# ztaylor797/APMBackend

Measured on AMD Instinct MI355X. Metric: log-lines/sec z-scored (whole node), higher is better.
Workload: dtype fp64

## Files before the change

### apmbackend_amd/csrc/bindings.cpp

```cpp
#include <pybind11/pybind11.h>
#include <pybind11/stl.h>

#include <cstring>
#include <memory>

#include "kernels/kernel_api.h"
#include "runtime/engine.h"
#include "runtime/format.h"
#include "runtime/jsutil.h"
#include "runtime/merge.h"

namespace apm {
namespace copyenc {
void encode_blob(std::string_view blob, std::string* out, int64_t* counts);
}
int apm_txcopy_lines(const char* d_text, const uint64_t* h_line_off, int64_t n, std::string& out_rows);
std::vector<double> apm_release_bench(int64_t n, int iters, uint64_t seed);
}

namespace py = pybind11;
using namespace apm;

void register_tailer(py::module_& m);
void register_synth(py::module_& m);
// ... 42 lines not shown
  c.max_lines = get<uint32_t>(d, "max_lines", c.max_lines);
  c.max_chunks = get<uint32_t>(d, "max_chunks", c.max_chunks);
  c.pool_cap = get<int64_t>(d, "pool_cap", c.pool_cap);
  c.max_tx_per_batch = get<int32_t>(d, "max_tx_per_batch", c.max_tx_per_batch);
  c.max_alerts = get<int32_t>(d, "max_alerts", c.max_alerts);
  c.ring_bytes = get<int>(d, "ring_bytes", c.ring_bytes);
  c.exact_mean = get<int>(d, "exact_mean", c.exact_mean);
  c.sigma_stddev = get<int>(d, "sigma_stddev", c.sigma_stddev);
  c.resync_k = get<int>(d, "resync_k", c.resync_k);
  c.resync_mfma = get<bool>(d, "resync_mfma", c.resync_mfma);
  c.emulate_aliasing = get<int>(d, "emulate_aliasing", c.emulate_aliasing);
  if (d.contains("lags")) {
    auto lags = d["lags"].cast<std::vector<std::tuple<int, double, double>>>();
    c.n_lags = (int)std::min<size_t>(lags.size(), MAX_LAGS);
    for (int i = 0; i < c.n_lags; ++i) {
      c.lags[i] = std::get<0>(lags[i]);
      c.thr[i] = std::get<1>(lags[i]);
      c.infl[i] = std::get<2>(lags[i]);
    }
  }
  if (d.contains("lag_suppressed")) {
    auto v = d["lag_suppressed"].cast<std::vector<int>>();
    for (size_t i = 0; i < v.size() && i < MAX_LAGS; ++i) c.lag_suppressed[i] = v[i];
  }
  c.alert_window = get<int>(d, "alert_window", c.alert_window);
  c.alert_threshold = get<int>(d, "alert_threshold", c.alert_threshold);
  c.hard_min_ms = get<double>(d, "hard_min_ms", c.hard_min_ms);
  c.hard_min_tpm = get<double>(d, "hard_min_tpm", c.hard_min_tpm);
  c.hard_max_ms = get<double>(d, "hard_max_ms", c.hard_max_ms);
  c.both_only = get<int>(d, "both_only", c.both_only);
  c.cooldown_ms = get<double>(d, "cooldown_ms", c.cooldown_ms);
  c.cooldown_by_service = get<int>(d, "cooldown_by_service", c.cooldown_by_service);
  c.alert_clock_entry = get<int>(d, "alert_clock_entry", c.alert_clock_entry);
  c.interval_len = get<int>(d, "interval_len", c.interval_len);
  c.window = get<int>(d, "window", c.window);
  c.buffer = get<int>(d, "buffer", c.buffer);
  c.nslot = get<int>(d, "nslot", c.nslot);
  c.ck_stage_bytes = get<int64_t>(d, "ck_stage_bytes", c.ck_stage_bytes);
  c.record_ttl_ms = get<double>(d, "record_ttl_ms", c.record_ttl_ms);
  c.acct_ttl_ms = get<double>(d, "acct_ttl_ms", c.acct_ttl_ms);
  c.need_ttl_ms = get<double>(d, "need_ttl_ms", c.need_ttl_ms);
  c.tz = tz_from(d);
  c.join_threads = get<int>(d, "join_threads", c.join_threads);
  c.pin_threads = get<bool>(d, "pin_threads", c.pin_threads);
  c.coll_timeout_ms = get<double>(d, "coll_timeout_ms", c.coll_timeout_ms);
  c.coll_init_timeout_ms = get<double>(d, "coll_init_timeout_ms", c.coll_init_timeout_ms);
  c.node_cooldown = get<int>(d, "node_cooldown", c.node_cooldown);
  c.outputs = get<uint32_t>(d, "outputs", c.outputs);
  if (d.contains("win_pcts")) {
    auto v = d["win_pcts"].cast<std::vector<int64_t>>();
    if (v.size() > 8) throw std::invalid_argument("win_pcts: at most 8 percentiles");
    c.n_win_pcts = (int32_t)v.size();
    for (size_t i = 0; i < v.size(); ++i) {
      if (v[i] < 1 || v[i] > 100000 || (i && v[i] <= v[i - 1]))
        throw std::invalid_argument("win_pcts: strictly ascending integers in 1 .. 100000 (percentile * 1000)");
      c.win_pcts[i] = (int32_t)v[i];
    }
  }
  if (d.contains("slo_classes")) {
    c.slo_classes = d["slo_classes"].cast<std::vector<std::vector<int64_t>>>();
    if (d.contains("slo_services")) c.slo_services = d["slo_services"].cast<std::map<std::string, int32_t>>();
    c.slo_default = get<int32_t>(d, "slo_default", 0);
  }
  if (d.contains("svc_pcts")) {
    auto v = d["svc_pcts"].cast<std::vector<int64_t>>();
    if (v.size() > 8) throw std::invalid_argument("svc_pcts: at most 8 percentiles");
    c.n_svc_pcts = (int32_t)v.size();
    for (size_t i = 0; i < v.size(); ++i) {
      if (v[i] < 1 || v[i] > 100000 || (i && v[i] <= v[i - 1]))
        throw std::invalid_argument("svc_pcts: strictly ascending integers in 1 .. 100000 (percentile * 1000)");
      c.svc_pcts[i] = (int32_t)v[i];
    }
  }
  if (d.contains("tk_k") && !d["tk_k"].is_none()) {
    c.tk_k = d["tk_k"].cast<int32_t>();
    if (d.contains("tk_by")) c.tk_by = d["tk_by"].cast<std::vector<int32_t>>();
    c.tk_min_tpm = get<double>(d, "tk_min_tpm", 0.0);
  }
  c.async_stats = get<int>(d, "async_stats", c.async_stats);
  c.device_join = get<int>(d, "device_join", c.device_join);
  c.join_table_bits = get<int>(d, "join_table_bits", c.join_table_bits);
  c.need_arena = get<uint32_t>(d, "need_arena", c.need_arena);
  c.join_chain_blocks = get<uint32_t>(d, "join_chain_blocks", c.join_chain_blocks);
  c.tx_ring_bytes = get<uint64_t>(d, "tx_ring_bytes", c.tx_ring_bytes);
  c.max_raw_services = get<uint32_t>(d, "max_raw_services", c.max_raw_services);
  return c;
}

ServiceOverride override_from(const py::dict& d) {
  ServiceOverride o;
  if (d.contains("thr")) {
    auto v = d["thr"].cast<std::vector<py::object>>();
    for (size_t i = 0; i < v.size() && i < MAX_LAGS; ++i)
      if (!v[i].is_none()) { o.has_thr[i] = true; o.thr[i] = v[i].cast<double>(); }
  }
  if (d.contains("infl")) {
    auto v = d["infl"].cast<std::vector<py::object>>();
    for (size_t i = 0; i < v.size() && i < MAX_LAGS; ++i)
      if (!v[i].is_none()) { o.has_infl[i] = true; o.infl[i] = v[i].cast<double>(); }
  }
  o.hard_max = get<double>(d, "hard_max", 0.0);
  o.suppressed = get<bool>(d, "suppressed", false);
  return o;
}

std::vector<Chunk> chunks_from(const std::vector<std::tuple<int32_t, uint64_t, uint64_t>>& v) {
  std::vector<Chunk> out;
  out.reserve(v.size());
  for (auto& t : v) out.push_back(Chunk{std::get<0>(t), std::get<1>(t), std::get<2>(t)});
  return out;
}

py::dict metrics_dict(const EngineMetrics& m) {
  py::dict d;
  d["batches"] = m.batches; d["bytes"] = m.bytes; d["lines"] = m.lines; d["events"] = m.events;
  d["tx"] = m.tx; d["tx_db"] = m.tx_db; d["tx_dropped"] = m.tx_dropped; d["rollovers"] = m.rollovers;
  d["alerts"] = m.alerts; d["alert_candidates"] = m.alert_candidates;
  d["alert_candidates_dropped"] = m.alert_candidates_dropped; d["released"] = m.released;
  d["staged_batches"] = m.staged_batches;
  d["t_join_shards_ms"] = m.t_join_shards_ms; d["t_merge_ms"] = m.t_merge_ms;
  d["t_shard_busy_ms"] = m.t_shard_busy_ms; d["t_shard_max_ms"] = m.t_shard_max_ms;
  d["t_out_ms"] = m.t_out_ms;
  d["t_lockstep_ms"] = m.t_lockstep_ms; d["t_lockstep_max_ms"] = m.t_lockstep_max_ms;
  d["t_lockstep_stats_ms"] = m.t_lockstep_stats_ms;
  d["db_copy_rows"] = m.db_copy_rows; d["db_copy_fallbacks"] = m.db_copy_fallbacks;
  d["t_stats_tx_ms"] = m.t_stats_tx_ms; d["t_rollover_ms"] = m.t_rollover_ms;
  d["t_format_ms"] = m.t_format_ms; d["t_release_ms"] = m.t_release_ms;
  d["formatted_bytes"] = m.formatted_bytes; d["lockstep_rollovers"] = m.lockstep_rollovers; d["format_fallbacks"] = m.format_fallbacks;
  d["t_parse_ms"] = m.t_parse_ms; d["t_join_ms"] = m.t_join_ms; d["t_stats_ms"] = m.t_stats_ms;
  d["t_total_ms"] = m.t_total_ms;
  d["series_overflow_tx"] = m.series_overflow_tx;
  d["spill_dropped"] = m.spill_dropped;
  d["nan_windows_clipped"] = m.nan_windows_clipped;
  d["tx_capacity_grows"] = m.tx_capacity_grows;
  d["spill_grows"] = m.spill_grows;
  d["spill_capacity"] = m.spill_capacity;
  d["rollover_latency_ms"] = m.rollover_latency_ms;
  return d;
}

py::dict counters_dict(const JoinCounters& c) {
  py::dict d;
  d["events"] = c.events; d["tx"] = c.tx; d["tx_db"] = c.tx_db; d["expired_partials"] = c.expired_partials;
  d["need_expired"] = c.need_expired; d["ejb_exit_unmatched"] = c.ejb_exit_unmatched;
  d["invalid_acct"] = c.invalid_acct; d["audit_errors"] = c.audit_errors; d["host_fallback"] = c.host_fallback;
  d["partial_overflow"] = c.partial_overflow; d["need_overflow"] = c.need_overflow; d["table_full"] = c.table_full;
  d["pool_exhausted"] = c.pool_exhausted; d["chain_partial_blocks"] = c.chain_partial_blocks;
  d["chain_need_blocks"] = c.chain_need_blocks; d["chain_logid_blocks"] = c.chain_logid_blocks;
  d["table_slots"] = c.table_slots; d["table_grows"] = c.table_grows; d["table_rebuilds"] = c.table_rebuilds; d["trims"] = c.trims;
  d["need_arena_entries"] = c.need_arena_entries; d["arena_grows"] = c.arena_grows;
  d["chain_pool_blocks"] = c.chain_pool_blocks; d["pool_grows"] = c.pool_grows;
  d["host_events"] = c.host_events;
  return d;
}

class JoinHarness {
 public:
  explicit JoinHarness(const py::dict& d) {
    cfg_.record_ttl_ms = get<double>(d, "record_ttl_ms", 120000);
    cfg_.acct_ttl_ms = get<double>(d, "acct_ttl_ms", 120000);
    cfg_.need_ttl_ms = get<double>(d, "need_ttl_ms", 30000);
    cfg_.tz = tz_from(d);
  }
  int32_t add_file(const std::string& path, int kind, const std::string& server) {
    int32_t sid;
    auto it = server_ids_.find(server);
    if (it == server_ids_.end()) {
      sid = (int32_t)servers_.size();
      servers_.push_back(server);
      server_ids_[server] = sid;
      shards_.emplace_back(new JoinShard(cfg_, &dict_, &files_, &servers_));
    } else {
      sid = it->second;
    }
    files_.push_back(FileInfo{path, sid, (uint8_t)kind});
    return (int32_t)files_.size() - 1;
  }
  std::vector<std::pair<std::string, std::string>> process(py::bytes events, py::bytes batch,
                                                           std::vector<int32_t> chunk_file, double now) {
    std::string ev = events;
    std::string by = batch;
    const Event* e = reinterpret_cast<const Event*>(ev.data());
    const size_t n = ev.size() / sizeof(Event);
    std::vector<std::pair<uint32_t, uint32_t>> range(shards_.size(), {0, 0});
    uint32_t i = 0;
    while (i < n) {
      const int32_t srv = files_[chunk_file[e[i].chunk]].server;
      uint32_t j = i;
      while (j < n && files_[chunk_file[e[j].chunk]].server == srv) ++j;
      range[srv] = {i, j};
      i = j;
    }
    std::vector<std::pair<std::string, std::string>> out;
    std::vector<TxOut> all;
    for (size_t s = 0; s < shards_.size(); ++s) {
      shards_[s]->out().clear();
      shards_[s]->begin_batch(now, batch_no_);
      if (range[s].second > range[s].first)
        shards_[s]->process(e + range[s].first, range[s].second - range[s].first, (const uint8_t*)by.data(),
                            chunk_file);
      for (auto& t : shards_[s]->out()) all.push_back(t);
    }
// ... 477 lines not shown
        rv.erase(rv.begin() + j);
      }
      if (sv.size() != rv.size() || !std::equal(rv.begin(), rv.end(), sv.begin())) return false;
    }
    return true;
  });
  m.def("gpu_to_fixed", [](const std::vector<double>& xs, int f, const std::string& mode) {
    const int md = mode == "nf" ? 0 : mode == "json" ? 1 : mode == "copy" ? 2 : -1;
    if (md < 0) throw std::invalid_argument("gpu_to_fixed: mode is nf, json or copy");
    if (f != 1 && f != 2) throw std::invalid_argument("gpu_to_fixed: f is 1 or 2");
    const int n = (int)xs.size();
    std::vector<char> h((size_t)n * 32);
    DevMem dx((size_t)n * 8), dout(h.size());
    HIP_OK(hipMemcpy(dx.p, xs.data(), (size_t)n * 8, hipMemcpyHostToDevice));
    apm_format_fixed_batch(dx.as<double>(), n, f, md, dout.as<char>(), 0);
    HIP_OK(hipMemcpy(h.data(), dout.p, h.size(), hipMemcpyDeviceToHost));
    std::vector<std::string> r;
    for (int i = 0; i < n; ++i) r.emplace_back(h.data() + (size_t)i * 32);
    return r;
  }, py::arg("xs"), py::arg("f"), py::arg("mode") = "nf");
  m.def("gpu_fleet_rows", [](const std::vector<double>& moments, const std::vector<std::string>& names,
                             const std::vector<int32_t>& lag_values, int32_t slot_lo, int32_t n_slots, bool copy,
                             int64_t edge_ts) {
    const int n_lags = (int)lag_values.size();
    if (n_lags < 1 || n_lags > MAX_LAGS) throw std::invalid_argument("gpu_fleet_rows: 1..MAX_LAGS lag values");
    if (slot_lo < 0 || n_slots < 0 || (size_t)slot_lo + (size_t)n_slots > names.size())
      throw std::invalid_argument("gpu_fleet_rows: slots outside names");
    if (moments.size() != names.size() * (size_t)n_lags * NSTAT * 3)
      throw std::invalid_argument("gpu_fleet_rows: moments hold names x lags x 3 x 3 doubles");
    std::vector<int32_t> nm;
    std::string chars;
    size_t longest = 0;
    for (const std::string& s : names) {
      nm.push_back((int32_t)chars.size());
      nm.push_back((int32_t)s.size());
      chars += s;
      longest = std::max(longest, s.size());
    }
    const int32_t rows = n_slots * n_lags;
    const uint32_t blocks = apm_fleet_format_blocks(rows);
    const size_t cap = apm_fleet_out_bound(rows, longest);
    DevMem m_mom(moments.size() * 8), m_nm(nm.size() * 4), m_out(cap);
    DevMem m_chars(chars.size() + 64);
    DevMem m_status((size_t)blocks * 8 + 64);
    double* d_mom = m_mom.as<double>();
    int32_t* d_nm = m_nm.as<int32_t>();
    char *d_chars = m_chars.as<char>(), *d_out = m_out.as<char>();
    unsigned long long* d_status = m_status.as<unsigned long long>();
    HIP_OK(hipMemset(d_chars, 0, chars.size() + 64));
    HIP_OK(hipMemset(d_status, 0, (size_t)blocks * 8 + 64));
    HIP_OK(hipMemcpy(d_mom, moments.data(), moments.size() * 8, hipMemcpyHostToDevice));
    HIP_OK(hipMemcpy(d_nm, nm.data(), nm.size() * 4, hipMemcpyHostToDevice));
    if (!chars.empty()) HIP_OK(hipMemcpy(d_chars, chars.data(), chars.size(), hipMemcpyHostToDevice));
    FleetFormatArgs fa{};
    fa.moments = d_mom;
    fa.names = reinterpret_cast<const int2*>(d_nm);
    fa.chars = d_chars;
    fa.slot_lo = slot_lo;
    fa.n_slots = n_slots;
    fa.n_lags = n_lags;
    std::vector<int> order(n_lags);
    for (int l = 0; l < n_lags; ++l) order[l] = l;
    std::sort(order.begin(), order.end(), [&](int a, int b) { return lag_values[a] < lag_values[b]; });
    for (int l = 0; l < n_lags; ++l) { fa.lag_order[l] = order[l]; fa.lag_value[l] = lag_values[l]; }
    fa.edge_ts = edge_ts;
    fa.copy = copy ? 1 : 0;
    fa.ts_len = Engine::pg_timestamp(edge_ts, fa.ts);
    fa.status = d_status;
    fa.total = reinterpret_cast<uint32_t*>(d_status + blocks);
    fa.out = d_out;
    fa.fallback = reinterpret_cast<int32_t*>(d_status + blocks) + 1;
    apm_fleet_format(&fa, 0);
    uint32_t total = 0;
    HIP_OK(hipMemcpy(&total, fa.total, 4, hipMemcpyDeviceToHost));
    if (total > cap) throw std::runtime_error("gpu_fleet_rows: rows longer than the output bound");
    std::string out(total, '\0');
    if (total) HIP_OK(hipMemcpy(&out[0], d_out, total, hipMemcpyDeviceToHost));
    return py::bytes(out);
  }, py::arg("moments"), py::arg("names"), py::arg("lag_values"), py::arg("slot_lo"), py::arg("n_slots"),
     py::arg("copy"), py::arg("edge_ts"));
  m.def("js_to_fixed", [](double x, int f) { return js::to_fixed(x, f); });
  m.def("js_num_str", [](double x) { return js::num_str(x); });
  m.def("js_parse_int", [](const std::string& s) { return js::parse_int(s); });
  m.def("js_convert_date", [](const std::string& s, const py::dict& tz) {
    double v;
    TzTable t = tz_from(tz);
    if (!js::convert_date(s, t, v)) return py::object(py::none());
    return py::object(py::float_(v));
  });
  m.def("js_round_fixed", [](double x, int f) { return js_round_fixed(x, f); });
  m.def("hist_bin", [](int32_t v) { return hist_bin(v); });
  m.def("hist_lower", [](int b) { return hist_lower(b); });
  m.def("hist_group_max", []() { return apm_hist_group_max(); });
  m.def("winpct_group_max", []() { return apm_winpct_group_max(); });
  m.def("winpct_group_win", []() { return apm_winpct_group_win(); });
  m.def("slo_group_max", []() { return apm_slo_group_max(); });
  m.def("slo_stage_bytes", []() { return apm_slo_stage_bytes(); });
  m.def("svcwin_group_max", []() { return apm_svcwin_group_max(); });
  m.def("svcwin_group_win", []() { return apm_svcwin_group_win(); });
  m.def("apm_topk_tile", []() { return apm_topk_tile(); });
  m.def("apm_topk_final_span", []() { return apm_topk_final_span(); });
  m.def("topk_select", [](const std::vector<std::tuple<double, double, double, double, int32_t>>& win_rows,
                          const std::vector<int32_t>& perm, int32_t k, const std::vector<int32_t>& by, double min_tpm) {
    if (k < 1 || k > TK_MAX_K) throw std::invalid_argument("topk_select: k is 1 .. 128");
    if (by.empty() || by.size() > (size_t)TK_MAX_BOARDS) throw std::invalid_argument("topk_select: 1 to 4 boards");
    for (int32_t c : by)
      if (c < TK_TPM || c > TK_P95) throw std::invalid_argument("topk_select: keys are 0 .. 3");
    for (int32_t s : perm)
      if (s < 0 || (size_t)s >= win_rows.size()) throw std::invalid_argument("topk_select: perm names no series");
    const int32_t n = (int32_t)perm.size(), S = (int32_t)win_rows.size(), nb = (int32_t)by.size();
    std::vector<WinStat> win((size_t)S);
    for (int32_t s = 0; s < S; ++s) {
      win[s].tpm = std::get<0>(win_rows[s]); win[s].avg = std::get<1>(win_rows[s]);
      win[s].p75 = std::get<2>(win_rows[s]); win[s].p95 = std::get<3>(win_rows[s]);
      win[s].n = 0; win[s].active = std::get<4>(win_rows[s]);
    }
    DevMem dwin((size_t)S * sizeof(WinStat)), dperm((size_t)n * 4), dsc(apm_topk_scratch_bytes(n, k, nb));
    DevMem dout((size_t)nb * k * sizeof(TopKRec)), dn(64);
    if (S) HIP_OK(hipMemcpy(dwin.p, win.data(), (size_t)S * sizeof(WinStat), hipMemcpyHostToDevice));
    if (n) HIP_OK(hipMemcpy(dperm.p, perm.data(), (size_t)n * 4, hipMemcpyHostToDevice));
    TopKArgs a{};
    a.win = dwin.as<WinStat>(); a.perm = dperm.as<int32_t>(); a.n = n; a.n_series = S; a.k = k; a.nb = nb;
    for (int32_t b = 0; b < nb; ++b) a.by[b] = by[b];
    a.min_tpm = min_tpm;
    a.out = dout.as<TopKRec>(); a.out_n = dn.as<int32_t>();
    apm_topk(&a, dsc.p, 0);
    std::vector<TopKRec> rec((size_t)nb * k);
    int32_t cnt[TK_MAX_BOARDS] = {0, 0, 0, 0};
    HIP_OK(hipMemcpy(cnt, dn.p, (size_t)nb * 4, hipMemcpyDeviceToHost));
    HIP_OK(hipMemcpy(rec.data(), dout.p, rec.size() * sizeof(TopKRec), hipMemcpyDeviceToHost));
    py::list out;
    for (int32_t b = 0; b < nb; ++b) {
      py::list rows;
      for (int32_t r = 0; r < std::min(std::max(cnt[b], 0), k); ++r)
        rows.append(py::make_tuple(rec[(size_t)b * k + r].series, rec[(size_t)b * k + r].pos));
      out.append(rows);
    }
    return out;
  }, py::arg("win_rows"), py::arg("perm"), py::arg("k"), py::arg("by"), py::arg("min_tpm") = 0.0);

  register_tailer(m);
  register_synth(m);
  register_procstat(m);
  register_dbsink(m);
}
```

### apmbackend_amd/csrc/kernels/kernel_api.h

```cpp
#pragma once
#include <hip/hip_runtime.h>
#include <stdint.h>

#include "../apm_types.h"
#include "common.h"

namespace apm {

struct StatsState {
  int32_t* counts;
  int32_t* cells;
  int32_t* spill_n;
  int32_t* spill_series;
  int32_t* spill_val;
  uint8_t* active;
  int32_t cap;
  int32_t spill_cap;
  int32_t S;
  int32_t nslot = NSLOT_MIN;
  unsigned long long* spill_drop = nullptr;
  int32_t* nan_until = nullptr;
  int32_t* ord_list = nullptr;
  int32_t* ord_n = nullptr;
  uint32_t* ord_done = nullptr;
// ... 205 lines not shown
struct TopKRec {
  int32_t series, pos;
  WinStat w;
};
struct TopKArgs {
  const WinStat* win;
  const int32_t* perm;
  int32_t n;
  int32_t n_series;
  int32_t k;
  int32_t nb;
  int32_t by[TK_MAX_BOARDS];
  double min_tpm;
  TopKRec* out;
  int32_t* out_n;
  int32_t tiles;
  uint64_t* sc_key;
  int32_t* sc_pos;
};
struct SvcRec {
  int32_t servers;
  int32_t m, nan;
  int32_t first_pos;
  long long sum;
  long long sum2[WP_MAX_Q];
};
struct SvcWinArgs {
  WindowArgs w;
  int32_t nq;
  int32_t q[WP_MAX_Q];
  int32_t n_groups;
  const int32_t* grp_off;
  const int32_t* grp_mem;
  const int32_t* grp_pos;
  SvcRec* rec;
  int32_t* big_list;
  int32_t* big_n;
};
struct SvcWinTextArgs {
  const SvcRec* rec;
  const int32_t* series_grp;
  const int32_t* perm;
  const int4* series_names;
  const char* names;
  int32_t n;
  int32_t n_series;
  int32_t n_groups;
  int32_t nq;
  int32_t ts_len;
  char ts[24];
  char ptxt[WP_MAX_Q][8];
  int32_t plen[WP_MAX_Q];
  uint32_t *len, *off;
  char* out;
};
struct AlertArgs {
  const WinStat* win;
  const ZOut* z;
  int32_t* counter;
  const double* hard_max;
  const uint8_t* suppressed;
  const uint64_t* emit_key;
  AlertRec* out;
  int32_t* n_out;
  int32_t n_series;
  int32_t lag_idx;
  int32_t n_lags;
  int32_t lag_suppressed;
  int32_t window;
  int32_t threshold;
  double hard_min_ms;
  double hard_min_tpm;
  int32_t both_only;
  int32_t max_out;
  const double* cool_t;
  double now;
  double cool_s;
};

}

extern "C" {
size_t apm_parse_workspace_bytes(uint64_t max_bytes, uint32_t max_lines, uint32_t max_chunks);
int apm_parse_batch(const uint8_t* d_bytes, uint64_t n_bytes, const uint32_t* d_chunk_begin,
                    const uint8_t* d_chunk_kind, const uint32_t* d_chunk_file, uint32_t n_chunks,
                    void* d_ws, uint32_t max_lines, apm::Event* d_events, uint32_t* d_n_events,
                    uint32_t* d_n_lines, unsigned long long* d_watermark, uint8_t* d_file_open,
                    const apm::TzTable* tz, hipStream_t stream);
size_t apm_ck_pack_tmp_bytes(uint64_t n_entries);
int apm_ck_pack_cells(const int32_t* counts, const int32_t* cells, const int32_t* d_slots, int k, int32_t n, int32_t S,
                      int32_t cap, uint32_t* lens, uint32_t* offs, void* tmp, size_t tmp_bytes, int32_t* packed,
                      hipStream_t s);
void apm_stats_clear_slot(apm::StatsState* st, int slot, hipStream_t stream);
void apm_bucket_append(const apm::TxRec* d_tx, uint32_t lo, uint32_t hi, apm::StatsState* st,
                       int64_t min_live_bucket, hipStream_t stream);
void apm_nan_mark(const apm::TxRec* d_tx, uint32_t n, apm::StatsState* st, hipStream_t stream);
void apm_window_stats(apm::WindowArgs* a, hipStream_t stream);
size_t apm_spill_sort_tmp_bytes(int32_t spill_cap, int32_t S, int32_t nslot);
int apm_spill_sort(const apm::StatsState* st, int32_t* series_out, int32_t* val_out, void* tmp, size_t tmp_bytes,
                   hipStream_t stream);
void apm_pool_append(const apm::TxRec* d_tx, uint32_t lo, uint32_t hi, const int64_t* d_gid, int64_t* tail_end,
                     int64_t* tail_gid, int64_t base, hipStream_t stream);
size_t apm_release_tmp_bytes(int64_t cap);
int apm_release_merge(const int64_t* pool_end, const int64_t* pool_gid, int64_t n_pool, const int64_t* tail_end,
                      const int64_t* tail_gid, int64_t n_tail, int64_t* sort_end, int64_t* sort_gid,
                      int64_t* out_end, int64_t* out_gid, void* tmp, size_t tmp_bytes, hipStream_t stream);
void apm_export(const apm::ExportArgs* a, hipStream_t stream);
void apm_copy(void* dst, const void* src, size_t bytes, hipStream_t stream);
void apm_copy_capped(void* dst, const void* src, size_t bytes, uint32_t max_blocks, hipStream_t stream);
void apm_copy_segs(const apm::CopySegs* c, hipStream_t stream);
void apm_set_f64(double* dst, const double* vals, int n, hipStream_t stream);
void apm_zscore(apm::ZArgs* a, int dtype_bytes, hipStream_t stream);
void apm_zscore_warm(apm::ZArgs* a, int dtype_bytes, int fill, uint64_t seed, const apm::WinStat* base,
                     hipStream_t stream);
void apm_server_rollup(apm::RollupArgs* a, hipStream_t stream);
size_t apm_format_tmp_bytes(int32_t n_max);
void apm_format_fixed_batch(const double* d_x, int n, int f, int mode, char* d_out, hipStream_t stream);
int apm_format_plan(apm::FormatArgs* a, void* tmp, size_t tmp_bytes, hipStream_t stream);
void apm_format_write(apm::FormatArgs* a, hipStream_t stream);
void apm_alert_eval(apm::AlertArgs* a, hipStream_t stream);
void apm_scatter_f64(double* dst, const int32_t* idx, const double* val, int32_t n, hipStream_t stream);
uint32_t apm_fleet_format_blocks(int32_t n_rows);
size_t apm_fleet_out_bound(int32_t rows, size_t longest);
void apm_fleet_format(apm::FleetFormatArgs* a, hipStream_t stream);
void apm_alert_gather(const apm::AlertRec* alerts, const int32_t* n_dev, int32_t max_n, const apm::WinStat* win,
                      const apm::ZOut* const* z_by_lag, int32_t n_lags, int32_t rows, apm::AlertRec* alerts_out,
                      apm::WinStat* win_out, apm::ZOut* z_out, int32_t* n_out, hipStream_t stream);
int32_t apm_hist_group_max();
size_t apm_hist_tmp_bytes(int32_t n_max);
size_t apm_hist_row_bound(size_t name_bytes);
int apm_hist_plan(apm::HistArgs* a, void* tmp, size_t tmp_bytes, hipStream_t stream);
void apm_hist_write(apm::HistArgs* a, hipStream_t stream);
int32_t apm_winpct_group_max();
int32_t apm_winpct_group_win();
size_t apm_winpct_tmp_bytes(int32_t n_max);
size_t apm_winpct_row_bound(size_t name_bytes, int32_t nq);
void apm_winpct_values(apm::WinPctArgs* a, hipStream_t stream);
int apm_winpct_plan(apm::WinPctTextArgs* a, void* tmp, size_t tmp_bytes, hipStream_t stream);
void apm_winpct_write(apm::WinPctTextArgs* a, hipStream_t stream);
int32_t apm_slo_group_max();
int32_t apm_slo_stage_bytes();
size_t apm_slo_tmp_bytes(int32_t n_max);
size_t apm_slo_row_bound(size_t name_bytes);
void apm_slo_values(apm::SloArgs* a, hipStream_t stream);
int apm_slo_plan(apm::SloTextArgs* a, void* tmp, size_t tmp_bytes, hipStream_t stream);
void apm_slo_write(apm::SloTextArgs* a, hipStream_t stream);
int32_t apm_topk_tile();
int32_t apm_topk_final_span();
size_t apm_topk_scratch_bytes(int32_t n_max, int32_t k, int32_t nb);
void apm_topk(apm::TopKArgs* a, void* scratch, hipStream_t stream);
int32_t apm_svcwin_group_max();
int32_t apm_svcwin_group_win();
size_t apm_svcwin_tmp_bytes(int32_t n_max);
size_t apm_svcwin_row_bound(size_t name_bytes, int32_t nq);
void apm_svcwin_values(apm::SvcWinArgs* a, hipStream_t stream);
int apm_svcwin_plan(apm::SvcWinTextArgs* a, void* tmp, size_t tmp_bytes, hipStream_t stream);
void apm_svcwin_write(apm::SvcWinTextArgs* a, hipStream_t stream);
void apm_service_moments(const int32_t* series_service, const uint8_t* active, int32_t n_series, int32_t S,
                         int32_t n_lags, int32_t n_services_cap, const double* const* sums, const double* const* comps,
                         const int32_t* const* cnts, double* dst, hipStream_t stream);
void apm_service_moments_tail(const int32_t* series_service, const uint8_t* active, int32_t s_lo, int32_t n_series,
                              int32_t S, int32_t n_lags, int32_t n_services_cap, const double* const* sums,
                              const double* const* comps, const int32_t* const* cnts, double* dst,
                              hipStream_t stream);
int apm_service_gram(const int32_t* svc_off, const int32_t* svc_ids, const uint8_t* active, int32_t n_services,
                     int32_t S, int32_t n_lags, const double* const* sums, const double* const* comps,
                     const int32_t* const* cnts, double* dst, hipStream_t stream, const int32_t* svc_map = nullptr,
                     int32_t accumulate = 0);
}
```

### apmbackend_amd/csrc/kernels/parse.hip

```cpp
#include "kernel_api.h"

#include "prim.h"

#include "devscan.h"

#include <algorithm>
#include <cstdio>
#include <cstdlib>
#include <cstring>

namespace apm {

constexpr int NL_BLOCK = 256;
constexpr int NL_TILE = NL_BLOCK * 16;
constexpr int PARSE_BLOCK = 256;
constexpr int PARSE_LDS = 32 * 1024;

constexpr int NL_PER = 4;

__device__ __forceinline__ uint32_t nl_count16(const uint4 v) {
  const uint32_t w[4] = {v.x, v.y, v.z, v.w};
  uint32_t c = 0;
#pragma unroll
  for (int k = 0; k < 4; ++k) {
    const uint32_t x = w[k] ^ 0x0a0a0a0aU;
    const uint32_t t = ~(((x & 0x7F7F7F7Fu) + 0x7F7F7F7Fu) | x | 0x7F7F7F7Fu);
    c += __popc(t);
  }
  return c;
}

__global__ __launch_bounds__(NL_BLOCK) void k_nl_count(const uint8_t* __restrict__ bytes, uint64_t n,
                                                      uint32_t* __restrict__ tile_counts, uint8_t* __restrict__ pad,
                                                      uint32_t tiles) {
  if (blockIdx.x == 0 && threadIdx.x < 64) pad[threadIdx.x] = 0;
  if (blockIdx.x == 0 && threadIdx.x == 64) tile_counts[tiles] = 0;
  uint4 v[NL_PER];
  uint64_t base[NL_PER];
#pragma unroll
  for (int k = 0; k < NL_PER; ++k) {
    base[k] = ((uint64_t)blockIdx.x * NL_PER + k) * NL_TILE + threadIdx.x * 16;
    if (base[k] + 16 <= n) v[k] = *reinterpret_cast<const uint4*>(bytes + base[k]);
  }
  uint32_t pk[NL_PER / 2] = {0, 0};
#pragma unroll
  for (int k = 0; k < NL_PER; ++k) {
    uint32_t c = 0;
    if (base[k] + 16 <= n) {
      c = nl_count16(v[k]);
    } else {
      for (uint64_t i = base[k]; i < n && i < base[k] + 16; ++i) c += bytes[i] == '\n';
    }
    pk[k >> 1] += c << (16 * (k & 1));
  }
  __shared__ uint32_t red[NL_PER / 2][NL_BLOCK / APM_WAVE];
#pragma unroll
  for (int h = 0; h < NL_PER / 2; ++h) {
    uint32_t c = pk[h];
    for (int o = 32; o > 0; o >>= 1) c += __shfl_down(c, o, APM_WAVE);
    if ((threadIdx.x & 63) == 0) red[h][threadIdx.x >> 6] = c;
  }
  __syncthreads();
  if (threadIdx.x < NL_PER) {
    const int k = threadIdx.x;
    uint32_t sum = 0;
    for (int i = 0; i < NL_BLOCK / APM_WAVE; ++i) sum += red[k >> 1][i];
    const uint32_t tile = blockIdx.x * NL_PER + k;
    if (tile < tiles) tile_counts[tile] = (sum >> (16 * (k & 1))) & 0xFFFFu;
  }
}

__global__ __launch_bounds__(NL_BLOCK) void k_nl_write(const uint8_t* __restrict__ bytes, uint64_t n,
                                                      const uint32_t* __restrict__ tile_off,
                                                      uint32_t* __restrict__ line_end, uint32_t* __restrict__ n_lines,
                                                      uint32_t tiles) {
  if (blockIdx.x == 0 && threadIdx.x == 0) *n_lines = tile_off[tiles];
  uint4 v[NL_PER];
#pragma unroll
  for (int k = 0; k < NL_PER; ++k) {
    const uint64_t base = ((uint64_t)blockIdx.x * NL_PER + k) * NL_TILE + threadIdx.x * 16;
    v[k] = base + 16 <= n ? *reinterpret_cast<const uint4*>(bytes + base) : make_uint4(0, 0, 0, 0);
  }
  typedef rocprim::block_scan<int, NL_BLOCK> Scan;
  __shared__ typename Scan::storage_type st;
#pragma unroll
  for (int k = 0; k < NL_PER; ++k) {
    const uint32_t tile = blockIdx.x * NL_PER + k;
    if (tile >= tiles) break;
    const uint64_t base = (uint64_t)tile * NL_TILE + threadIdx.x * 16;
    uint8_t b[16];
    if (base + 16 <= n) {
      const uint32_t w[4] = {v[k].x, v[k].y, v[k].z, v[k].w};
#pragma unroll
      for (int q = 0; q < 4; ++q) {
#pragma unroll
        for (int j = 0; j < 4; ++j) b[q * 4 + j] = (uint8_t)(w[q] >> (8 * j));
      }
    } else {
      for (int i = 0; i < 16; ++i) b[i] = (base + i < n) ? bytes[base + i] : 0;
    }
    int c = 0;
#pragma unroll
    for (int i = 0; i < 16; ++i) c += b[i] == '\n';
    int excl;
    Scan().exclusive_scan(c, excl, 0, st);
    uint32_t pos = tile_off[tile] + excl;
#pragma unroll
    for (int i = 0; i < 16; ++i)
      if (b[i] == '\n') line_end[pos++] = (uint32_t)(base + i);
    __syncthreads();
  }
}

__device__ __forceinline__ bool is_ws(uint8_t c) {
  return c <= 32 && ((0x100003E00ULL >> c) & 1ULL);
}
__device__ __forceinline__ bool is_digit(uint8_t c) { return c >= '0' && c <= '9'; }
__device__ __forceinline__ uint8_t lower(uint8_t c) { return (c >= 'A' && c <= 'Z') ? c + 32 : c; }

template <int N>
__device__ __forceinline__ bool match_at(const uint8_t* p, int i, int len, const char (&lit)[N]) {
  if (i + N - 1 > len) return false;
#pragma unroll
  for (int k = 0; k < N - 1; ++k)
    if (p[i + k] != (uint8_t)lit[k]) return false;
  return true;
}

constexpr int NTOKSLOT = 7;
__device__ __forceinline__ constexpr int tok_slot(int k) {
  return k <= 3 ? k : (k == 9 ? 4 : (k == 11 ? 5 : (k == 13 ? 6 : 0)));
}
__device__ __forceinline__ void tok_put(uint16_t (&arr)[NTOKSLOT], int k, uint16_t v) {
  constexpr int idx[NTOKSLOT] = {0, 1, 2, 3, 9, 11, 13};
#pragma unroll
  for (int j = 0; j < NTOKSLOT; ++j) arr[j] = k == idx[j] ? v : arr[j];
}
__device__ __forceinline__ void tok_put_if(uint16_t (&arr)[NTOKSLOT], bool on, int k, uint16_t v) {
  tok_put(arr, on ? k : -1, v);
}
constexpr uint64_t kTokSlotTab = 0xFF6F5F4FFFFF3210ULL;
__device__ __forceinline__ int tok_slot_of(int k) { return k < 16 ? (int)((kTokSlotTab >> (4 * k)) & 0xFu) : 15; }

template <int N>
__device__ __forceinline__ constexpr uint32_t pk4(const char (&lit)[N]) {
  static_assert(N == 5, "pk4 takes exactly four characters");
  return (uint32_t)(uint8_t)lit[0] | ((uint32_t)(uint8_t)lit[1] << 8) | ((uint32_t)(uint8_t)lit[2] << 16) |
         ((uint32_t)(uint8_t)lit[3] << 24);
}

__device__ __forceinline__ uint32_t swar_eq(uint32_t d, uint32_t k4) {
  const uint32_t x = d ^ k4;
  return ~(((x & 0x7F7F7F7Fu) + 0x7F7F7F7Fu) | x | 0x7F7F7F7Fu);
}
__device__ __forceinline__ uint32_t swar_ws(uint32_t d) {
  const uint32_t y = d & 0x7F7F7F7Fu;
  const uint32_t rng = (y + 0x77777777u) & ~(y + 0x72727272u) & ~d & 0x80808080u;
  return rng | swar_eq(d, 0x20202020u);
}
__device__ __forceinline__ uint32_t swar_bits(uint32_t t) { return (((t >> 7) * 0x00204081u) >> 21) & 0xFu; }

struct Masks16 {
  uint32_t ws, na, trig;
};
__device__ __forceinline__ Masks16 masks16(const uint32_t (&d)[5]) {
  Masks16 r{0u, 0u, 0u};
#pragma unroll
  for (int q = 0; q < 4; ++q) {
    r.ws |= swar_bits(swar_ws(d[q])) << (4 * q);
    r.na |= swar_bits(d[q] & 0x80808080u) << (4 * q);
// ... 22 lines not shown
  if (i < e && (p[i] == '+' || p[i] == '-')) { neg = p[i] == '-'; ++i; }
  if (i + 1 < e && p[i] == '0' && (p[i + 1] == 'x' || p[i + 1] == 'X')) return false;
  int64_t v = 0;
  int nd = 0;
  while (i < e && is_digit(p[i])) {
    v = v * 10 + (p[i] - '0');
    ++i;
    if (++nd > 15) return false;
  }
  out = nd == 0 ? apm_nan() : (neg ? -(double)v : (double)v);
  return true;
}

__device__ inline bool parse_log_ts(const uint8_t* p, int s1, int e1, int s2, int e2,
                                    const TzTable& tz, double& out, bool& strict) {
  int64_t v[8];
  int np = 0;
  int nd[8];
  strict = false;
  for (int pass = 0; pass < 2; ++pass) {
    const int s = pass ? s2 : s1, e = pass ? e2 : e1;
    int64_t cur = 0;
    int cnt = 0;
    for (int i = s; i <= e; ++i) {
      const bool end = i == e;
      const uint8_t c = end ? '-' : p[i];
      if (c == '-' || c == ':' || c == ',') {
        if (np >= 8) return false;
        v[np] = cur; nd[np] = cnt; ++np;
        cur = 0; cnt = 0;
        if (end) break;
      } else if (is_digit(c)) {
        cur = cur * 10 + (c - '0');
        if (++cnt > 12) return false;
      } else {
        return false;
      }
    }
  }
  if (np < 7) {
    out = apm_nan();
    return np >= 2;
  }
  const int64_t yr = (v[0] >= 0 && v[0] <= 99) ? v[0] + 1900 : v[0];
  const int64_t local = make_date_ms(yr, v[1] - 1, v[2], v[3], v[4], v[5], v[6]);
  out = (double)local_to_utc(tz, local);
  strict = np == 7 && nd[0] == 4 && nd[1] == 2 && nd[2] == 2 && nd[3] == 2 && nd[4] == 2 &&
           nd[5] == 2 && nd[6] >= 1 && nd[6] <= 3;
  return true;
}

__device__ __forceinline__ bool parse_log_ts_fixed(const uint8_t* p, int s1, int e1, int s2, int e2,
                                                   const TzTable& tz, double& out) {
  if (e1 - s1 != 10 || e2 - s2 != 12) return false;
  uint32_t a[10], b[12];
#pragma unroll
  for (int k = 0; k < 10; ++k) a[k] = (uint32_t)p[s1 + k] - '0';
#pragma unroll
  for (int k = 0; k < 12; ++k) b[k] = (uint32_t)p[s2 + k] - '0';
  bool ok = a[4] == (uint32_t)('-' - '0') && a[7] == (uint32_t)('-' - '0') && b[2] == (uint32_t)(':' - '0') &&
            b[5] == (uint32_t)(':' - '0') && b[8] == (uint32_t)(',' - '0');
  constexpr int da[8] = {0, 1, 2, 3, 5, 6, 8, 9};
  constexpr int db[9] = {0, 1, 3, 4, 6, 7, 9, 10, 11};
#pragma unroll
  for (int k = 0; k < 8; ++k) ok &= a[da[k]] <= 9u;
#pragma unroll
  for (int k = 0; k < 9; ++k) ok &= b[db[k]] <= 9u;
  if (!ok) return false;
  const int64_t y = a[0] * 1000 + a[1] * 100 + a[2] * 10 + a[3];
  const int64_t mo = a[5] * 10 + a[6], d = a[8] * 10 + a[9];
  const int64_t h = b[0] * 10 + b[1], mi = b[3] * 10 + b[4], sec = b[6] * 10 + b[7];
  const int64_t ms = b[9] * 100 + b[10] * 10 + b[11];
  const int64_t yr = y <= 99 ? y + 1900 : y;
  out = (double)local_to_utc(tz, make_date_ms(yr, mo - 1, d, h, mi, sec, ms));
  return true;
}

struct ParseArgs {
  const uint8_t* bytes;
  const uint32_t* line_end;
  const uint32_t* chunk_begin;
  const uint8_t* chunk_kind;
  const uint32_t* n_lines_dev;
  uint32_t cap_lines;
  uint32_t n_chunks;
  Event* ev_tmp;
  uint32_t* line_mask;
  uint8_t* keep;
  unsigned long long* watermark;
  unsigned long long* prof;
  TzTable tz;
};

enum : int { PP_STAGE = 0, PP_SCAN, PP_HITS, PP_LINES, PP_WAVES, PP_COOP, PP_SERIAL, PP_HEAD, PP_TAIL, PP_N = 10 };
__device__ __forceinline__ void pprof(const ParseArgs& a, int k, long long& t) {
  if (a.prof) {
    const long long now = clock64();
    if ((threadIdx.x & (APM_WAVE - 1)) == 0) atomicAdd(&a.prof[k], (unsigned long long)(now - t));
    t = now;
  }
}

__device__ __forceinline__ uint32_t find_chunk_in(const uint32_t* cb, uint32_t lo, uint32_t hi, uint32_t pos) {
  while (lo < hi) {
    uint32_t mid = (lo + hi + 1) >> 1;
    if (cb[mid] <= pos) lo = mid; else hi = mid - 1;
  }
  return lo;
}

__device__ __forceinline__ uint32_t find_chunk(const uint32_t* cb, uint32_t n_chunks, uint32_t pos) {
  uint32_t lo = 0, hi = n_chunks - 1;
  while (lo < hi) {
    uint32_t mid = (lo + hi + 1) >> 1;
    if (cb[mid] <= pos) lo = mid; else hi = mid - 1;
  }
  return lo;
}

template <int STRIDE = PARSE_BLOCK>
__device__ __forceinline__ unsigned long long parse_line(const ParseArgs& a, const uint8_t* __restrict__ base,
                                                         uint32_t o, uint32_t li, uint32_t ls, uint32_t le,
                                                         uint32_t c_lo, uint32_t c_hi, uint16_t* tp);

enum : uint32_t { XF_EJB_ENTRY = 1, XF_EJB_EXIT = 2, XF_CT_START = 4, XF_CT_STOP = 8, XF_BAF = 16, XF_NONASCII = 32 };

template <class P>
__device__ __forceinline__ void probe_flags(P p, int len, int s, uint32_t& m, uint32_t& xf) {
  const uint32_t w4 = (uint32_t)p[s] | ((uint32_t)p[s + 1] << 8) | ((uint32_t)p[s + 2] << 16) |
                      ((uint32_t)p[s + 3] << 24);
  if (w4 == pk4("INFO")) {
    int j = s + 4;
    while (j < len && p[j] == ' ') ++j;
    if (match_at(p, j, len, "[CommonTiming] The EJB")) xf |= XF_EJB_ENTRY;
    if (match_at(p, j, len, "[CommonTiming] Total time")) xf |= XF_EJB_EXIT;
    if (match_at(p, j, len, "CommonTiming::Start")) xf |= XF_CT_START;
    if (match_at(p, j, len, "CommonTiming::Stop")) xf |= XF_CT_STOP;
    if (match_at(p, s, len, "INFO  auditTrailId=")) m |= PM_AUTR_MAP;
    if (!(xf & XF_BAF) && s + 4 < len && p[s + 4] == ' ' && s >= 1 && p[s - 1] == ' ') {
      int kk0 = s - 1;
      while (kk0 >= 0 && p[kk0] == ' ') --kk0;
      if (kk0 >= 0 && p[kk0] == ']')
        for (int kk = kk0 - 2; kk >= 0 && p[kk] != ' '; --kk)
          if (p[kk] == '[') { xf |= XF_BAF; break; }
    }
    return;
  }
  if (w4 == pk4(": Re")) {
    if (match_at(p, s, len, ": RequestTrace [stopWatchList=")) m |= PM_EL_START;
    return;
  }
  if ((w4 & 0xffu) != '<') return;
  const uint32_t w4l = (uint32_t)lower(p[s]) | ((uint32_t)lower(p[s + 1]) << 8) |
                       ((uint32_t)lower(p[s + 2]) << 16) | ((uint32_t)lower(p[s + 3]) << 24);
  if (w4 == pk4("<sto")) {
    if (match_at(p, s, len, "<stopWatchList>")) m |= PM_SW_START;
    if (match_at(p, s, len, "<stopTime>")) m |= PM_SW_STOPTS;
  } else if (w4 == pk4("</st")) {
    if (match_at(p, s, len, "</stopWatchList>")) m |= PM_SW_END;
  } else if (w4 == pk4("<nam")) {
    if (match_at(p, s, len, "<name>")) m |= PM_SW_NAME;
  } else if (w4 == pk4("<sta")) {
    if (match_at(p, s, len, "<startTime>")) m |= PM_SW_STARTTS;
  } else if (w4 == pk4("<val")) {
    if (match_at(p, s, len, "<value>")) m |= PM_SOAP_VALUE;
  }
  if (w4l == pk4("<acc")) {
    if (match_at_ci(p, s, len, "<accountnumber>")) m |= PM_SOAP_ACCT;
  } else if (w4l == pk4("<key")) {
    if (match_at_ci(p, s, len, "<key>accountnumber</key>")) m |= PM_SOAP_KEY;
  }
}

template <int STRIDE>
__device__ __forceinline__ unsigned long long line_tail(const ParseArgs& a, const uint8_t* __restrict__ p, int len,
                                                        uint32_t li, Event& ev, uint8_t fk, int ntok, uint32_t m,
                                                        uint32_t xf, int info1, int info2, const uint16_t* tp,
                                                        int bias);
__device__ __forceinline__ bool line_head(const ParseArgs& a, const uint8_t* __restrict__ p, uint32_t li,
                                          uint32_t ls, uint32_t le, uint32_t c_lo, uint32_t c_hi, Event& ev,
                                          uint8_t& fk, int& len);

__global__ __launch_bounds__(PARSE_BLOCK) void k_parse_lines(ParseArgs a) {
  __shared__ __attribute__((aligned(16))) uint8_t lds[PARSE_LDS];
  __shared__ uint16_t tok_lds[2 * NTOKSLOT][PARSE_BLOCK];
  long long pt = a.prof ? clock64() : 0;
  const uint32_t n_lines = *a.n_lines_dev;
  const uint32_t first = blockIdx.x * PARSE_BLOCK;
  if (first >= n_lines) {
    const uint32_t li = first + threadIdx.x;
    if (li < a.cap_lines) a.keep[li] = 0;
    return;
  }
  const uint32_t last = min(first + PARSE_BLOCK, n_lines);
  const uint32_t r0 = first == 0 ? 0 : a.line_end[first - 1] + 1;
  const uint32_t r1 = a.line_end[last - 1] + 1;
  const uint32_t a0 = r0 & ~15u;
  const uint32_t span = r1 - a0;
  const bool staged = span <= PARSE_LDS;
  if (staged) {
    const uint32_t nvec = (span + 15) >> 4;
    const uint4* __restrict__ src = reinterpret_cast<const uint4*>(a.bytes + a0);
    uint4* dst = reinterpret_cast<uint4*>(lds);
    const uint32_t t = threadIdx.x;
    for (uint32_t i = t; i < nvec; i += 4 * PARSE_BLOCK) {
      const bool b1 = i + PARSE_BLOCK < nvec, b2 = i + 2 * PARSE_BLOCK < nvec, b3 = i + 3 * PARSE_BLOCK < nvec;
      const uint4 v0 = src[i];
      const uint4 v1 = b1 ? src[i + PARSE_BLOCK] : v0;
      const uint4 v2 = b2 ? src[i + 2 * PARSE_BLOCK] : v0;
      const uint4 v3 = b3 ? src[i + 3 * PARSE_BLOCK] : v0;
      dst[i] = v0;
      if (b1) dst[i + PARSE_BLOCK] = v1;
      if (b2) dst[i + 2 * PARSE_BLOCK] = v2;
      if (b3) dst[i + 3 * PARSE_BLOCK] = v3;
    }
  }
  __syncthreads();
  pprof(a, PP_STAGE, pt);
  const uint32_t li = first + threadIdx.x;
  unsigned long long wm = 0;
  if (li >= last) {
    if (li < a.cap_lines) a.keep[li] = 0;
  } else {
    const uint32_t ls = li == 0 ? 0 : a.line_end[li - 1] + 1;
    const uint32_t le = a.line_end[li];
    const uint32_t c_lo = find_chunk(a.chunk_begin, a.n_chunks, r0), c_hi = find_chunk(a.chunk_begin, a.n_chunks, r1 - 1);
    wm = staged ? parse_line<PARSE_BLOCK>(a, lds, ls - a0, li, ls, le, c_lo, c_hi, &tok_lds[0][threadIdx.x])
                : parse_line<PARSE_BLOCK>(a, a.bytes, ls, li, ls, le, c_lo, c_hi, &tok_lds[0][threadIdx.x]);
  }
  if (a.prof) {
    pprof(a, PP_LINES, pt);
    if ((threadIdx.x & (APM_WAVE - 1)) == 0) atomicAdd(&a.prof[PP_WAVES], 1ull);
  }
  for (int off = APM_WAVE / 2; off > 0; off >>= 1) {
    const unsigned long long o2 = __shfl_xor(wm, off, APM_WAVE);
    wm = o2 > wm ? o2 : wm;
  }
  if ((threadIdx.x & (APM_WAVE - 1)) == 0 && wm) atomicMax(a.watermark, wm);
}

__device__ __forceinline__ bool line_head(const ParseArgs& a, const uint8_t* __restrict__ p, uint32_t li,
                                          uint32_t ls, uint32_t le, uint32_t c_lo, uint32_t c_hi, Event& ev,
                                          uint8_t& fk, int& len) {
  len = (int)(le - ls);
  if (len > 0 && p[len - 1] == '\r') --len;

  ev.line = li;
  ev.chunk = find_chunk_in(a.chunk_begin, c_lo, c_hi, ls);
  ev.off = ls;
  ev.len = (uint32_t)len;
  ev.mask = 0;
  ev.kind = LK_NONE;
  ev.ntok = 0;
  ev.pad0 = 0;
  ev.t0s = ev.t0e = ev.t1s = ev.t1e = ev.t2s = ev.t2e = ev.t3s = ev.t3e = 0xffff;
  ev.tAs = ev.tAe = ev.tBs = ev.tBe = 0xffff;
  ev.ts = apm_nan();
  ev.num = apm_nan();
  ev.key = 0;
  ev.svc = 0;
  fk = a.chunk_kind[ev.chunk];
  if (len <= 0 || len > 65000) {
    a.keep[li] = (len > 65000) ? 1 : 0;
    if (len > 65000) { ev.kind = fk == FILE_SOAP ? LK_SOAP : LK_APP; ev.mask = PM_HOST; }
    a.line_mask[li] = ev.mask;
    a.ev_tmp[li] = ev;
    return false;
  }
  return true;
}

constexpr int TILE = NL_TILE;
constexpr int TSTAGE = TILE + 1024;
constexpr int TMAXL = 128;
constexpr int THITS = 256;

__device__ __forceinline__ uint32_t tscan_op(uint32_t x, uint32_t y) {
  const uint32_t ls = (x & 0x1FFFu) + (y & 0x1FFFu);
  const uint32_t hits = (x >> 19) + (y >> 19);
  uint32_t seg, has;
  if (y & 0x2000u) {
    seg = (y >> 14) & 31u;
    has = 1u;
  } else {
    seg = min(((x >> 14) & 31u) + ((y >> 14) & 31u), 31u);
    has = (x >> 13) & 1u;
  }
  return ls | (has << 13) | (seg << 14) | (hits << 19);
}

__global__ __launch_bounds__(APM_WAVE) void k_parse_tiles(ParseArgs a, uint64_t n, const uint32_t* __restrict__ tile_off) {
  __shared__ __attribute__((aligned(16))) uint8_t st[TSTAGE + 32];
  __shared__ uint16_t tok[2 * NTOKSLOT][TMAXL];
  __shared__ uint16_t c_ls[TMAXL], c_le[TMAXL];
  __shared__ uint8_t c_nt[TMAXL];
  __shared__ uint32_t c_m[TMAXL], c_xf[TMAXL], c_i1[TMAXL], c_i2[TMAXL];
  __shared__ uint32_t hit[THITS];
  const int lane = threadIdx.x;
  long long pt = a.prof ? clock64() : 0;
  const uint32_t n_lines = *a.n_lines_dev;
  for (uint32_t li = n_lines + blockIdx.x * APM_WAVE + lane; li < a.cap_lines; li += gridDim.x * APM_WAVE)
    a.keep[li] = 0;
  const uint64_t T0 = (uint64_t)blockIdx.x * TILE;
  if (T0 >= n) return;
  const uint64_t T1 = min(T0 + TILE, n);
  const bool own0 = T0 == 0 || a.bytes[T0 - 1] == '\n';
// ... 473 lines not shown
    const unsigned long long cm = __ballot(is_close);
    const unsigned long long below = lane ? ((1ULL << lane) - 1ULL) : 0ULL;
    const unsigned long long ob = om & below, cb = cm & below;
    bool in;
    if (!ob && !cb) in = open;
    else {
      const int lo_ = ob ? 63 - __clzll(ob) : -1;
      const int lc_ = cb ? 63 - __clzll(cb) : -1;
      in = lo_ > lc_;
    }
    if (valid && in && !is_open) {
      line_mask[li] = m | PM_IN_SECTION;
      if (!keep[li]) {
        keep[li] = 1;
        ev_tmp[li].kind = LK_APP;
      }
      ev_tmp[li].mask |= PM_IN_SECTION;
    }
    const unsigned long long all = om | cm;
    if (all) {
      const int l = 63 - __clzll(all);
      open = (om >> l) & 1ULL;
    }
  }
  if (g == SEC_SEGS - 1 && lane == 0) {
    bool fin = chunk_init[c] != 0;
    for (int h = SEC_SEGS - 1; h >= 0; --h) {
      const uint8_t st = seg_state[(size_t)c * SEC_SEGS + h];
      if (st) { fin = st == 1; break; }
    }
    file_open[chunk_file[c]] = fin ? 1 : 0;
  }
}

__global__ void k_chunk_lines(const uint32_t* __restrict__ chunk_begin, uint32_t n_chunks,
                              const uint32_t* __restrict__ line_end, const uint32_t* __restrict__ n_lines_dev,
                              uint32_t* __restrict__ chunk_line_lo, const uint32_t* __restrict__ tile_off,
                              uint32_t tiles) {
  const uint32_t c = blockIdx.x * blockDim.x + threadIdx.x;
  if (c > n_chunks) return;
  const uint32_t n_lines = *n_lines_dev;
  const uint32_t pos = chunk_begin[c];
  const uint32_t t = pos / (uint32_t)NL_TILE;
  uint32_t lo = t < tiles ? tile_off[t] : n_lines, hi = t < tiles ? tile_off[t + 1] : n_lines;
  while (lo < hi) {
    uint32_t mid = (lo + hi) >> 1;
    if (line_end[mid] < pos) lo = mid + 1; else hi = mid;
  }
  chunk_line_lo[c] = lo;
}

struct KeepF {
  const uint8_t* keep;
  __device__ uint32_t operator()(uint32_t i) const { return keep[i]; }
};
struct CompactG {
  const uint8_t* keep;
  const Event* ev_tmp;
  Event* out;
  __device__ void operator()(uint32_t i, uint32_t p) const {
    if (keep[i]) out[p] = ev_tmp[i];
  }
};

}

extern "C" {

constexpr size_t APM_SCAN_TMP = 32u << 20;

size_t apm_parse_workspace_bytes(uint64_t max_bytes, uint32_t max_lines, uint32_t max_chunks) {
  using namespace apm;
  const uint64_t tiles = (max_bytes + NL_TILE - 1) / NL_TILE + 2;
  size_t b = 0;
  b += tiles * 8 + 64;
  b += (size_t)max_lines * (4 + 4 + 4 + 1) + 64;
  b += (size_t)max_lines * sizeof(Event) + 64;
  b += (size_t)(max_chunks + 2) * 4 + 256;
  b += (size_t)(max_chunks + 2) * (SEC_SEGS + 1) + 256;
  b += APM_SCAN_TMP;
  return b;
}

int apm_parse_batch(const uint8_t* d_bytes, uint64_t n_bytes, const uint32_t* d_chunk_begin,
                    const uint8_t* d_chunk_kind, const uint32_t* d_chunk_file, uint32_t n_chunks,
                    void* d_ws, uint32_t max_lines, apm::Event* d_events, uint32_t* d_n_events,
                    uint32_t* d_n_lines, unsigned long long* d_watermark, uint8_t* d_file_open,
                    const apm::TzTable* tz, hipStream_t stream) {
  using namespace apm;
  const uint32_t tiles = (uint32_t)((n_bytes + NL_TILE - 1) / NL_TILE);
  if (tiles == 0 || n_chunks == 0) {
    HIP_OK(hipMemsetAsync(d_n_events, 0, 4, stream));
    HIP_OK(hipMemsetAsync(d_n_lines, 0, 4, stream));
    HIP_OK(hipMemsetAsync(const_cast<uint8_t*>(d_bytes) + n_bytes, 0, 64, stream));
    return 0;
  }
  const uint32_t cap = (uint32_t)std::min<uint64_t>(max_lines, n_bytes);
  uint8_t* w = (uint8_t*)d_ws;
  auto carve = [&](size_t bytes) { uint8_t* r = (uint8_t*)(((uintptr_t)w + 63) & ~(uintptr_t)63); w = r + bytes; return r; };
  uint32_t* tile_counts = (uint32_t*)carve((size_t)(tiles + 1) * 4);
  uint32_t* tile_off = (uint32_t*)carve((size_t)(tiles + 1) * 4);
  uint32_t* line_end = (uint32_t*)carve((size_t)max_lines * 4);
  Event* ev_tmp = (Event*)carve((size_t)max_lines * sizeof(Event));
  uint32_t* line_mask = (uint32_t*)carve((size_t)max_lines * 4);
  uint32_t* pos = (uint32_t*)carve((size_t)max_lines * 4);
  uint8_t* keep = carve((size_t)max_lines);
  uint32_t* chunk_line_lo = (uint32_t*)carve((size_t)(n_chunks + 2) * 4);
  uint8_t* seg_state = carve((size_t)(n_chunks + 2) * SEC_SEGS);
  uint8_t* chunk_init = carve((size_t)(n_chunks + 2));
  void* scan_tmp = carve(APM_SCAN_TMP);

  const uint32_t nl_blocks = (tiles + NL_PER - 1) / NL_PER;
  hipLaunchKernelGGL(k_nl_count, dim3(nl_blocks), dim3(NL_BLOCK), 0, stream, d_bytes, n_bytes, tile_counts,
                     const_cast<uint8_t*>(d_bytes) + n_bytes, tiles);
  PrimScratch sc(scan_tmp, APM_SCAN_TMP);
  if (prim_exclusive_scan(sc, tile_counts, tile_off, 0u, (size_t)tiles + 1, rocprim::plus<uint32_t>(), stream) != 0)
    return -1;
  hipLaunchKernelGGL(k_nl_write, dim3(nl_blocks), dim3(NL_BLOCK), 0, stream, d_bytes, n_bytes, tile_off, line_end,
                     d_n_lines, tiles);

  ParseArgs pa;
  pa.bytes = d_bytes;
  pa.line_end = line_end;
  pa.chunk_begin = d_chunk_begin;
  pa.chunk_kind = d_chunk_kind;
  pa.n_lines_dev = d_n_lines;
  pa.cap_lines = cap;
  pa.n_chunks = n_chunks;
  pa.ev_tmp = ev_tmp;
  pa.line_mask = line_mask;
  pa.keep = keep;
  pa.watermark = d_watermark;
  pa.tz = *tz;
  static unsigned long long* d_prof = nullptr;
  static int prof_batches = 0;
  static const bool prof_on = getenv("APM_PARSE_PROF") != nullptr;
  if (prof_on && !d_prof) {
    HIP_OK(hipMalloc((void**)&d_prof, PP_N * 8));
    HIP_OK(hipMemsetAsync(d_prof, 0, PP_N * 8, stream));
  }
  pa.prof = prof_on ? d_prof : nullptr;
  const char* mode_env = getenv("APM_PARSE");
  const bool by_line = !(mode_env && strcmp(mode_env, "tile") == 0);
  if (by_line)
    hipLaunchKernelGGL(k_parse_lines, dim3((cap + PARSE_BLOCK - 1) / PARSE_BLOCK), dim3(PARSE_BLOCK), 0,
                       stream, pa);
  else
    hipLaunchKernelGGL(k_parse_tiles, dim3(tiles), dim3(APM_WAVE), 0, stream, pa, n_bytes, (const uint32_t*)tile_off);
  if (prof_on && ++prof_batches % 50 == 0) {
    unsigned long long h[PP_N];
    HIP_OK(hipMemcpyAsync(h, d_prof, sizeof h, hipMemcpyDeviceToHost, stream));
    HIP_OK(hipStreamSynchronize(stream));
    const double w = h[PP_WAVES] ? (double)h[PP_WAVES] : 1.0;
    fprintf(stderr, "[parse prof %s] %d batches, %.0f waves/batch; cycles per wave: stage %.0f scan %.0f hits %.0f "
            "lines %.0f; lines coop %llu serial %llu; per coop line: head %.0f tail %.0f\n", by_line ? "line" : "tile",
            prof_batches, w / prof_batches, h[PP_STAGE] / w, h[PP_SCAN] / w, h[PP_HITS] / w, h[PP_LINES] / w,
            (unsigned long long)h[PP_COOP], (unsigned long long)h[PP_SERIAL],
            h[PP_COOP] ? (double)h[PP_HEAD] / h[PP_COOP] : 0.0, h[PP_COOP] ? (double)h[PP_TAIL] / h[PP_COOP] : 0.0);
  }
  hipLaunchKernelGGL(k_chunk_lines, dim3((n_chunks + 1 + 255) / 256), dim3(256), 0, stream, d_chunk_begin,
                     n_chunks, line_end, d_n_lines, chunk_line_lo, tile_off, tiles);
  hipLaunchKernelGGL(k_section_summary, dim3(n_chunks, SEC_SEGS), dim3(APM_WAVE), 0, stream, chunk_line_lo,
                     d_chunk_kind, d_chunk_file, n_chunks, line_mask, d_file_open, seg_state, chunk_init);
  hipLaunchKernelGGL(k_section_apply, dim3(n_chunks, SEC_SEGS), dim3(APM_WAVE), 0, stream, chunk_line_lo,
                     d_chunk_kind, d_chunk_file, n_chunks, line_mask, keep, ev_tmp, d_file_open, seg_state,
                     chunk_init);
  if (ds_scan_apply<uint32_t>(KeepF{keep}, CompactG{keep, ev_tmp, d_events}, d_n_lines, cap, pos, d_n_events,
                              stream) != 0)
    return -1;
  return 0;
}

}
```

### apmbackend_amd/csrc/runtime/devjoin.h

```cpp
#pragma once
#include <hip/hip_runtime.h>

#include <atomic>
#include <cstdint>
#include <deque>
#include <functional>
#include <mutex>
#include <string>
#include <unordered_map>
#include <vector>

#include "../apm_types.h"
#include "../kernels/devjoin_api.h"
#include "hipres.h"
#include "join.h"

namespace apm {

struct CopySegs;

struct DevJoinConfig {
  uint32_t max_events = 1u << 20;
  uint64_t max_batch_bytes = 64ull << 20;
  uint32_t max_chunks = 4096;
  int table_bits = 21;
  int reg_bits = 20;
  uint32_t max_raw = 1u << 20;
  uint32_t arena_cap = 1u << 20;
  uint32_t pool_blocks = 0;
  uint64_t ring_bytes = 4ull << 30;
  double record_ttl_ms = 120000, acct_ttl_ms = 120000, need_ttl_ms = 30000;
  TzTable tz{};
  int device = 0;
};

struct DevJoinBatch {
  int slot = 0;
  uint32_t n_out = 0, n_stats = 0, n_db = 0, n_dropped = 0;
  std::vector<std::pair<uint32_t, int64_t>> cands;
  std::vector<std::pair<uint32_t, int32_t>> unresolved;
  std::string text_tx, text_db;
  uint64_t ring_base = 0;
  int64_t max_bucket = INT64_MIN;
  TxRec* d_tx = nullptr;
  int32_t* d_raw = nullptr;
  int64_t* d_gid = nullptr;
};

class DeviceJoin {
 public:
  DeviceJoin(const DevJoinConfig& cfg, Dictionary* dict, const std::vector<FileInfo>* files,
             const std::vector<std::string>* servers);
  ~DeviceJoin();

  uint8_t* d_bytes(int k) { return sl_[k].d_bytes; }
  uint8_t* d_stage() {
    if (!d_stage_bytes_) {
      d_stage_bytes_ = (uint8_t*)res_.dmalloc_on(stream_, cfg_.max_batch_bytes + 256);
      HIP_OK(hipStreamSynchronize(stream_));
    }
    return d_stage_bytes_;
  }
  void swap_stage(int k) { std::swap(sl_[k].d_bytes, d_stage_bytes_); }
  Event* d_events(int k) { return sl_[k].d_events; }
  void select_host(int k, const uint32_t* d_n_ev, uint32_t max_ev, hipStream_t ps);
  void set_chunks(int k, const std::vector<int32_t>& chunk_file, const uint32_t* d_chunk_file,
                  const uint8_t* d_chunk_kind);
  void chunk_upload(int k, uint32_t max_ev, CopySegs& cs);
  void export_select(int k, CopySegs& cs);
  using ParallelFor = std::function<void(int, const std::function<void(int)>&)>;
  void run(int k, const uint8_t* host_bytes, uint32_t n_ev, uint64_t n_bytes, double now, uint64_t batch_no, bool want_tx,
           bool want_db, DevJoinBatch& out, const ParallelFor& parallel = nullptr,
           const std::function<void()>* meanwhile = nullptr);
  void prepass_ahead(int k, const uint8_t* host_bytes, const ParallelFor& parallel);
  void release_slot(int k, hipStream_t stats_stream);

  int32_t raw_server(int32_t raw) const { return raw_info_[raw].server; }
  int32_t raw_service(int32_t raw) const { return raw_info_[raw].norm_id; }
  int32_t n_raw() const { return n_raw_.load(std::memory_order_acquire); }
  int32_t* d_raw_series() { return d_raw_series_; }

  char* ring() { return d_ring_; }
  uint64_t ring_cap() const { return cfg_.ring_bytes; }
  void set_ring_low(uint64_t low);
  uint64_t ring_head() const { return ring_head_.load(std::memory_order_acquire); }
  uint64_t ring_low() const { return ring_low_.load(std::memory_order_acquire); }
  uint64_t keys_live() const { return keys_live_ + keys_since_rebuild_; }
  uint64_t need_live() const { return arena_head_ - (regions_.empty() ? arena_head_ : regions_.front().lo); }
  uint64_t ring_reserve(uint64_t bytes);
  void reset_ring(uint64_t head);

  JoinCounters counters() const;
  std::vector<uint64_t> cache_stats(double now, bool sync = true);

  void save(class BinWriter& w);
  void load(class BinReader& r);
  static constexpr int kPhases = 8;
  double phase_t[kPhases + 1] = {0};
  std::vector<std::pair<const char*, std::pair<double, double>>> spans;
  std::vector<std::pair<const char*, std::pair<double, double>>> save_spans;
  const JoinCounts& last_counts() const { return *h_counts_; }
  size_t device_bytes() const { return res_.device_bytes(); }
  size_t trim(double now);

 private:
  struct Slot {
    uint8_t* d_bytes = nullptr;
    Event* d_events = nullptr;
    uint8_t* host_flag = nullptr;
    uint32_t* d_mh_idx = nullptr;
    uint32_t* d_walk_idx = nullptr;
    AudF* d_aud = nullptr;
    SelCount* d_n_host = nullptr;
    Mapped<Event> h_host_ev;
    Mapped<uint32_t> h_host_idx;
    Mapped<SelCount> h_n_host;
    int32_t* d_chunk_next = nullptr;
    uint8_t* d_chunk_first = nullptr;
    Mapped<int32_t> h_chunk_next;
    Mapped<uint8_t> h_chunk_first;
    const uint32_t* d_chunk_file = nullptr;
    const uint8_t* d_chunk_kind = nullptr;
    uint32_t n_chunks = 0;
    std::vector<int32_t> chunk_file;
    TxRec* d_tx = nullptr;
    int32_t* d_tx_raw = nullptr;
    int64_t* d_tx_gid = nullptr;
    hipEvent_t free_ev = nullptr;
    bool used = false;
  } sl_[2];

  struct RawInfo { int32_t server; int32_t norm_id; uint64_t svc; };

  struct PrepassTask {
    int32_t file = -1;
    std::vector<uint32_t> idx;
    std::vector<HostOp> hops;
    std::string hbuf;
    uint64_t audit_errors = 0, invalid_acct = 0, pm_host = 0;
    uint32_t put(std::string_view s) { const uint32_t o = (uint32_t)hbuf.size(); hbuf.append(s.data(), s.size()); return o; }
  };
  void host_prepass(int k, const uint8_t* host_bytes, uint32_t n_host, const ParallelFor& parallel,
                    std::vector<HostOp>& hops, std::string& hbuf);
  void host_event(PrepassTask& t, const Event& e, uint32_t ev, const uint8_t* host_bytes);
  void on_app(PrepassTask& t, const Event& e, uint32_t ev, std::string_view line);
  void save_tables(class BinWriter& w);
  void aud_reserve(AudGen& g, uint32_t autr, uint32_t items, uint64_t txt);
// ... 161 lines not shown
```

### apmbackend_amd/csrc/runtime/engine.cpp

```cpp
#include <cstdlib>
#include "engine.h"

#include <pthread.h>
#include <sched.h>

#include <cctype>
#include <fstream>

#include <rocprofiler-sdk-roctx/roctx.h>

#include <unistd.h>

#include <cerrno>
#include <cstring>

#include <algorithm>
#include <exception>
#include <chrono>
#include <cmath>
#include <cstring>
#include <queue>
#include <stdexcept>

#include "../kernels/devjoin_api.h"
// ... 163 lines not shown
  done_cv_.wait(lk, [&]() { return done_ == n_tasks_; });
  fn_ = nullptr;
  lk.unlock();
  if (err) std::rethrow_exception(err);
}

Engine::Engine(const EngineConfig& cfg) : cfg_(cfg) {
  check_window(cfg_.window, cfg_.buffer, cfg_.interval_len);
  if (cfg_.n_lags < 1 || cfg_.n_lags > MAX_LAGS)
    throw std::runtime_error("engine: 1.." + std::to_string(MAX_LAGS) + " LAG settings");
  if (want(OUT_WP)) {
    const int nq = cfg_.n_win_pcts;
    bool ok = nq >= 1 && nq <= WP_MAX_Q;
    for (int j = 0; ok && j < nq; ++j)
      ok = cfg_.win_pcts[j] >= 1 && cfg_.win_pcts[j] <= 100000 && (j == 0 || cfg_.win_pcts[j] > cfg_.win_pcts[j - 1]);
    if (!ok) throw std::invalid_argument("wp stream: win_pcts must hold 1 to 8 strictly ascending percentiles");
  }
  if (want(OUT_SL)) {
    const auto& cl = cfg_.slo_classes;
    bool ok = !cl.empty() && cl[0].empty() && cl.size() <= (size_t)cfg_.max_series + 2;
    bool any = false;
    for (size_t c = 1; ok && c < cl.size(); ++c) {
      ok = !cl[c].empty() && cl[c].size() <= (size_t)SL_MAX_T;
      for (size_t j = 0; ok && j < cl[c].size(); ++j)
        ok = cl[c][j] >= 0 && cl[c][j] <= INT32_MAX && (j == 0 || cl[c][j] > cl[c][j - 1]);
      any = true;
    }
    const auto in_range = [&](int32_t c) { return c >= 0 && (size_t)c < cl.size(); };
    ok = ok && any && in_range(cfg_.slo_default);
    for (const auto& kv : cfg_.slo_services) ok = ok && in_range(kv.second);
    if (!ok)
      throw std::invalid_argument("sl stream: slo_classes must hold the empty class 0 and at least one class of 1 to 8 "
                                  "strictly ascending thresholds in 0 .. 2147483647; every class index must name one");
  }
  if (want(OUT_TK)) {
    bool ok = cfg_.tk_k >= 1 && cfg_.tk_k <= TK_MAX_K && !cfg_.tk_by.empty() && cfg_.tk_by.size() <= (size_t)TK_MAX_BOARDS &&
              std::isfinite(cfg_.tk_min_tpm) && cfg_.tk_min_tpm >= 0.0;
    for (size_t i = 0; ok && i < cfg_.tk_by.size(); ++i) {
      ok = cfg_.tk_by[i] >= TK_TPM && cfg_.tk_by[i] <= TK_P95;
      for (size_t j = 0; ok && j < i; ++j) ok = cfg_.tk_by[j] != cfg_.tk_by[i];
    }
    if (!ok)
      throw std::invalid_argument("tk stream: tk_k must lie in 1 .. 128, tk_by hold 1 to 4 distinct keys out of "
                                  "0 .. 3 and tk_min_tpm be finite and >= 0");
  }
  if (want(OUT_SV)) {
    const int nq = cfg_.n_svc_pcts;
    bool ok = nq >= 1 && nq <= WP_MAX_Q;
    for (int j = 0; ok && j < nq; ++j)
      ok = cfg_.svc_pcts[j] >= 1 && cfg_.svc_pcts[j] <= 100000 && (j == 0 || cfg_.svc_pcts[j] > cfg_.svc_pcts[j - 1]);
    if (!ok) throw std::invalid_argument("sv stream: svc_pcts must hold 1 to 8 strictly ascending percentiles");
  }
  HIP_OK(hipSetDevice(cfg_.device));
  {
    const char* e = std::getenv("APM_BLOCKING_SYNC");
    if (e && e[0] == '1') (void)hipSetDeviceFlags(hipDeviceScheduleBlockingSync);
  }
  {
    const char* e = std::getenv("APM_CU_RESERVE");
    int n_cu = 0;
    HIP_OK(hipDeviceGetAttribute(&n_cu, hipDeviceAttributeMultiprocessorCount, cfg_.device));
    const int reserve = e ? std::atoi(e) : 0;
    if (reserve > 0 && reserve < n_cu / 2) {
      const int stride = n_cu / reserve;
      std::vector<uint32_t> mask((size_t)(n_cu + 31) / 32, 0u);
      for (int c = 0; c < n_cu; ++c)
        if (c % stride != stride - 1) mask[(size_t)c / 32] |= 1u << (c % 32);
      for (hipStream_t* s : {&stream_, &parse_stream_, &out_stream_})
        HIP_OK(hipExtStreamCreateWithCUMask(s, (uint32_t)mask.size(), mask.data()));
      cu_reserved_ = reserve;
    } else {
      static const bool sp = [] { const char* x = std::getenv("APM_STATS_PRIO"); return !(x && x[0] == '0'); }();
      int lo = 0, hi = 0;
      HIP_OK(hipDeviceGetStreamPriorityRange(&lo, &hi));
      HIP_OK(hipStreamCreateWithPriority(&stream_, hipStreamNonBlocking, sp ? hi : 0));
      static const bool pp = [] { const char* x = std::getenv("APM_PARSE_PRIO"); return x && x[0] == '1'; }();
      HIP_OK(hipStreamCreateWithPriority(&parse_stream_, hipStreamNonBlocking, pp ? hi : 0));
      HIP_OK(hipStreamCreateWithFlags(&out_stream_, hipStreamNonBlocking));
    }
    for (hipStream_t st : {stream_, parse_stream_, out_stream_}) res_.adopt(st);
  }
  ev_a_ = res_.new_event();
  ev_b_ = res_.new_event();
  const int32_t S = cfg_.max_series;
  if (cfg_.device_join) {
    DevJoinConfig dc;
    dc.max_events = cfg_.max_lines;
    dc.max_batch_bytes = cfg_.max_batch_bytes;
    dc.max_chunks = cfg_.max_chunks;
    dc.table_bits = cfg_.join_table_bits;
    dc.max_raw = cfg_.max_raw_services;
    dc.arena_cap = cfg_.need_arena;
    dc.pool_blocks = cfg_.join_chain_blocks;
    dc.ring_bytes = cfg_.tx_ring_bytes;
    dc.record_ttl_ms = cfg_.record_ttl_ms;
    dc.acct_ttl_ms = cfg_.acct_ttl_ms;
    dc.need_ttl_ms = cfg_.need_ttl_ms;
    dc.tz = cfg_.tz;
    dc.device = cfg_.device;
    dj_.reset(new DeviceJoin(dc, &dict_, &files_, &servers_));
    d_ring_min_ = (unsigned long long*)res_.dmalloc(64);
    HIP_OK(hipMemset(d_ring_min_, 0xff, 8));
    res_.pin(h_ring_min_, 64);
    *h_ring_min_ = ~0ULL;
    d_rel_n_ = (int64_t*)res_.dmalloc(64);
    res_.pin(h_rel_n_, 64);
    d_rel_lens_ = (uint32_t*)res_.dmalloc(((size_t)cfg_.pool_cap + 2) * 4);
    d_rel_offs_ = (uint32_t*)res_.dmalloc(((size_t)cfg_.pool_cap + 2) * 4);
    d_rel_fb_ = (uint32_t*)res_.dmalloc(4);
    HIP_OK(hipMemset(d_rel_fb_, 0, 4));
    res_.pin(h_rel_total_, 64);
    d_unmapped_ = (unsigned long long*)res_.dmalloc(64);
    d_unseen_idx_ = (int32_t*)res_.dmalloc((size_t)cfg_.max_series * 4);
    d_unseen_flag_ = (uint8_t*)res_.dmalloc((size_t)cfg_.max_series);
    res_.pin(h_unseen_flag_, (size_t)cfg_.max_series);
  } else {
    d_bytes_ = (uint8_t*)res_.dmalloc(cfg_.max_batch_bytes + 256);
  }
  for (int k = 0; k < 2; ++k) {
    ParseSlot& ps = pslot_[k];
    res_.pin(ps.h_bytes, cfg_.max_batch_bytes + 256);
    res_.pin(ps.h_chunk_begin, (cfg_.max_chunks + 2) * 4);
    res_.pin(ps.h_chunk_kind, cfg_.max_chunks + 2);
    res_.pin(ps.h_chunk_file, (cfg_.max_chunks + 2) * 4);
    d_chunk_begin_[k] = (uint32_t*)res_.dmalloc((cfg_.max_chunks + 2) * 4);
    d_chunk_kind_[k] = (uint8_t*)res_.dmalloc(cfg_.max_chunks + 2);
    d_chunk_file_[k] = (uint32_t*)res_.dmalloc((cfg_.max_chunks + 2) * 4);
    res_.pin(ps.h_counts, 16);
    res_.pin(ps.h_watermark, 8);
    if (dev()) continue;
    res_.pin(ps.h_events, (size_t)cfg_.max_lines * sizeof(Event));
  }
  d_parse_ws_ = res_.dmalloc(apm_parse_workspace_bytes(cfg_.max_batch_bytes, cfg_.max_lines, cfg_.max_chunks));
  if (!dev()) d_events_ = (Event*)res_.dmalloc((size_t)cfg_.max_lines * sizeof(Event));
  d_counts_ = (uint32_t*)res_.dmalloc(16);
  d_watermark_ = (unsigned long long*)res_.dmalloc(8);
  d_file_open_ = (uint8_t*)res_.dmalloc(1 << 16);
  init_spill_cap_ = cfg_.spill_cap;
  alloc_ring(std::max(cfg_.nslot, ring_slots_for(cfg_.window, cfg_.buffer)));
  for (auto& m : spill_mark_) m.ev = res_.new_event();
  metrics_.spill_capacity = cfg_.spill_cap;
  d_spill_drop_ = (unsigned long long*)res_.dmalloc(64);
  d_active_ = (uint8_t*)res_.dmalloc(S);
  d_win_ = (WinStat*)res_.dmalloc((size_t)S * sizeof(WinStat));
  d_big_list_ = (int32_t*)res_.dmalloc((size_t)S * 4);
  d_big_n_ = (int32_t*)res_.dmalloc(64);
  d_nan_until_ = (int32_t*)res_.dmalloc((size_t)S * 4);
  HIP_OK(hipMemset(d_nan_until_, 0x80, (size_t)S * 4));
  ord_cap_ = std::max<int64_t>(cfg_.max_tx_per_batch, cfg_.max_lines);
  d_ord_list_ = (int32_t*)res_.dmalloc((size_t)ord_cap_ * 4);
  d_ord_n_ = (int32_t*)res_.dmalloc(8);
  d_nan_list_ = (int32_t*)res_.dmalloc((size_t)S * 4);
  d_nan_n_ = d_big_n_ + 1;
  d_js_scratch_ = (int32_t*)res_.dmalloc((size_t)JS_BLOCKS * kJsCap * 4);
  for (int l = 0; l < cfg_.n_lags; ++l) {
    LagState& L = lag_[l];
    L.ring = res_.dmalloc((size_t)NSTAT * cfg_.lags[l] * S * cfg_.ring_bytes);
    L.len = (int32_t*)res_.dmalloc((size_t)S * 4);
    L.sum = (double*)res_.dmalloc((size_t)NSTAT * S * 8);
    L.comp = (double*)res_.dmalloc((size_t)NSTAT * S * 8);
    L.sumsq = (double*)res_.dmalloc((size_t)NSTAT * S * 8);
    L.sqcomp = (double*)res_.dmalloc((size_t)NSTAT * S * 8);
    L.cnt = (int32_t*)res_.dmalloc((size_t)NSTAT * S * 4);
    L.thr = (double*)res_.dmalloc((size_t)S * 8);
    L.infl = (double*)res_.dmalloc((size_t)S * 8);
    L.out = (ZOut*)res_.dmalloc((size_t)S * sizeof(ZOut));
// ... 88 lines not shown
    d_sv_len_ = (uint32_t*)res_.dmalloc((size_t)(S + 1) * 4);
    d_sv_off_txt_ = (uint32_t*)res_.dmalloc((size_t)(S + 1) * 4);
    sv_tmp_bytes_ = apm_svcwin_tmp_bytes(S);
    d_sv_tmp_ = res_.dmalloc(sv_tmp_bytes_);
    res_.pin(h_sv_total_, 64);
    for (int k = 0; k < 2; ++k) ev_sv_[k] = res_.new_event();
  }
  if (want(OUT_LH)) {
    d_hist_len_ = (uint32_t*)res_.dmalloc((size_t)(S + 1) * 4);
    d_hist_off_ = (uint32_t*)res_.dmalloc((size_t)(S + 1) * 4);
    d_hist_big_ = (int32_t*)res_.dmalloc((size_t)(S + 1) * 4);
    hist_tmp_bytes_ = apm_hist_tmp_bytes(S);
    d_hist_tmp_ = res_.dmalloc(hist_tmp_bytes_);
    res_.pin(h_hist_total_, 64);
    for (int k = 0; k < 2; ++k) ev_hist_[k] = res_.new_event();
  }
  {
    const char* f = std::getenv("APM_TXCOPY_FORCE_FALLBACK");
    txcopy_force_fb_ = f && f[0] == '1';
  }
  d_alerts_ = (AlertRec*)res_.dmalloc((size_t)cfg_.max_alerts * sizeof(AlertRec));
  d_n_alerts_ = d_big_n_ + 2;
  res_.pin(h_alerts_, (size_t)cfg_.max_alerts * sizeof(AlertRec));
  res_.pin(h_alert_win_, (size_t)cfg_.max_alerts * sizeof(WinStat));
  res_.pin(h_alert_z_, (size_t)cfg_.max_alerts * sizeof(ZOut));
  res_.pin(h_n_alerts_, 16);
  ev_alerts_ = res_.new_event();
  ev_release_ = res_.new_event();
  d_tx_ = (TxRec*)res_.dmalloc((size_t)cfg_.max_tx_per_batch * sizeof(TxRec));
  res_.pin(h_tx_, (size_t)cfg_.max_tx_per_batch * sizeof(TxRec));
  d_gid_ = (int64_t*)res_.dmalloc((size_t)cfg_.max_tx_per_batch * 8);
  res_.pin(h_gid_, (size_t)cfg_.max_tx_per_batch * 8);
  d_tail_end_ = (int64_t*)res_.dmalloc((size_t)cfg_.pool_cap * 8);
  d_tail_gid_ = (int64_t*)res_.dmalloc((size_t)cfg_.pool_cap * 8);
  d_sort_end_ = (int64_t*)res_.dmalloc((size_t)cfg_.pool_cap * 8);
  d_sort_gid_ = (int64_t*)res_.dmalloc((size_t)cfg_.pool_cap * 8);
  for (int i = 0; i < 2; ++i) {
    d_pool_end_[i] = (int64_t*)res_.dmalloc((size_t)cfg_.pool_cap * 8);
    d_pool_gid_[i] = (int64_t*)res_.dmalloc((size_t)cfg_.pool_cap * 8);
  }
  release_tmp_bytes_ = apm_release_tmp_bytes(cfg_.pool_cap);
  if (dev()) release_tmp_bytes_ = std::max(release_tmp_bytes_, apm_dj_tmp_bytes((uint32_t)cfg_.pool_cap + 2, 1024));
  d_release_tmp_ = res_.dmalloc(release_tmp_bytes_);
  for (int k = 0; k < 2; ++k) {
    res_.pin(h_release_gid_[k], (size_t)cfg_.pool_cap * 8);
    ev_rel_[k] = res_.new_event();
    ev_fmt_[k] = res_.new_event();
  }
  const char* pin_env = std::getenv("APM_PIN_THREADS");
  if (pin_env ? std::atoi(pin_env) != 0 : cfg_.pin_threads) lane_cpus_ = local_core_slice(cfg_.device);
  int nt = cfg_.join_threads;
  if (nt <= 0) nt = (int)std::min<unsigned>(cfg_.device_join ? 8 : 16, std::max(1u, std::thread::hardware_concurrency()));
  {
    std::vector<int> wc(lane_cpus_.begin(), lane_cpus_.begin() + (ptrdiff_t)std::min<size_t>(lane_cpus_.size(), (size_t)std::max(nt, 0)));
    pool_.reset(new ThreadPool(nt > 1 ? nt : 0, wc));
  }
  for (int l = 0; l < MAX_LAGS; ++l) { alias_thr_[l] = cfg_.thr[l]; alias_infl_[l] = cfg_.infl[l]; }
  HIP_OK(hipStreamSynchronize(stream_));
  HIP_OK(hipDeviceSynchronize());
  const int nt_used = std::max(cfg_.join_threads > 0 ? cfg_.join_threads : 0, pool_->size());
  const int st_cpu = (int)lane_cpus_.size() > nt_used ? lane_cpus_[nt_used] : -1;
  const int out_cpu = (int)lane_cpus_.size() > nt_used + 1 ? lane_cpus_[nt_used + 1] : -1;
  roll_lane_mode_ = !want(OUT_SX);
  if (roll_lane_mode_) roll_lane_.reset(new TaskLane());
  stats_thread_ = std::thread([this, st_cpu]() {
    if (st_cpu >= 0) pin_current_thread(st_cpu);
    hipSetDevice(cfg_.device);
    stats_worker();
  });
  out_thread_ = std::thread([this, out_cpu]() {
    if (out_cpu >= 0) pin_current_thread(out_cpu);
    hipSetDevice(cfg_.device);
    out_worker();
  });
}

Engine::~Engine() {
  if (roll_lane_) {
    try { roll_lane_->wait_all(); } catch (...) {}
    roll_lane_.reset();
  }
  ahead_lane_.reset();
  if (in_stage_stream_) hipStreamSynchronize(in_stage_stream_);
  fb_lane_.reset();
  if (nm_ev_) hipEventSynchronize(nm_ev_);
  checkpoint_shutdown();
  {
    std::lock_guard<std::mutex> g(st_mu_);
    st_stop_ = true;
  }
  st_cv_.notify_all();
  if (stats_thread_.joinable()) stats_thread_.join();
  {
    std::lock_guard<std::mutex> g(out_mu_);
    out_stop_ = true;
  }
  out_cv_.notify_all();
  if (out_thread_.joinable()) out_thread_.join();
  if (rel_lane_) {
    try { rel_lane_->wait_all(); } catch (...) {}
    rel_lane_.reset();
  }
  if (coll_) {
    hipStreamSynchronize(coll_stream_);
    coll_.reset();
    if (fb_stream_) hipStreamSynchronize(fb_stream_);
  }
  hipStreamSynchronize(stream_);
  hipStreamSynchronize(parse_stream_);
  auto wait_holds = [this](int idx, void* slot) {
    FmtHolds& hs = *fmt_holds_;
    std::unique_lock<std::mutex> lk(hs.mu);
    if (!hs.cv.wait_for(lk, std::chrono::seconds(60), [&] { return hs.n[idx] == 0; })) res_.forget(slot);
  };
  for (int r = 0; r < FMT_RING; ++r) wait_holds(6 + r, h_fmt_ring_[r].p);
  for (int k = 0; k < 2; ++k) wait_holds(2 + k, h_fb_out_[k].p);
  if (cool_ev_) hipEventSynchronize(cool_ev_);
  if (dj_) {
    hipStreamSynchronize(out_stream_);
    for (int r = 0; r < REL_RING; ++r) wait_holds(6 + FMT_RING + r, h_rel_text_[r].p);
    dj_.reset();
  }
  hipStreamSynchronize(out_stream_);
  if (rel_stream_) hipStreamSynchronize(rel_stream_);
  res_.release_all();
}

int32_t Engine::add_server(const std::string& name) {
  flush();
  auto it = server_ids_.find(name);
  if (it != server_ids_.end()) return it->second;
  const int32_t id = (int32_t)servers_.size();
  servers_.push_back(name);
  server_ids_[name] = id;
  server_rank_.push_back(-1);
  server_next_service_.push_back(0);
  server_gidx_.push_back(id);
  server_first_batch_.push_back(-1);
  JoinConfig jc;
  jc.record_ttl_ms = cfg_.record_ttl_ms;
  jc.acct_ttl_ms = cfg_.acct_ttl_ms;
  jc.need_ttl_ms = cfg_.need_ttl_ms;
  jc.tz = cfg_.tz;
  shards_.emplace_back(new JoinShard(jc, &dict_, &files_, &servers_));
  return id;
}

int32_t Engine::add_file(const std::string& path, int kind, const std::string& server) {
  flush();
  const int32_t sid = add_server(server);
  files_.push_back(FileInfo{path, sid, (uint8_t)kind});
  if (files_.size() > (1 << 16)) throw std::runtime_error("too many files");
  return (int32_t)files_.size() - 1;
}

void Engine::set_override(const std::string& service, const ServiceOverride& o) {
  flush();
  overrides_[service] = o;
}
void Engine::clear_overrides() {
  flush();
  overrides_.clear();
}

void Engine::compute_series_settings(int32_t s, double* thr, double* infl, double& hard_max, uint8_t& suppressed) {
  const std::string& svc = dict_.service_name(series_[s].service);
// ... 160 lines not shown
  if (dj_) return dj_->counters();
  JoinCounters t;
  for (auto& s : shards_) {
    const JoinCounters& c = s->counters;
    t.events += c.events; t.tx += c.tx; t.tx_db += c.tx_db; t.expired_partials += c.expired_partials;
    t.need_expired += c.need_expired; t.ejb_exit_unmatched += c.ejb_exit_unmatched;
    t.invalid_acct += c.invalid_acct; t.audit_errors += c.audit_errors; t.host_fallback += c.host_fallback;
  }
  return t;
}

void Engine::launch_parse(ParseSlot& ps, const uint8_t* host_bytes, uint64_t n_bytes, const std::vector<Chunk>& chunks_in,
                          bool speculative) {
  const double t0 = now_ms();
  if (n_bytes > cfg_.max_batch_bytes) throw std::runtime_error("batch larger than max_batch_bytes");
  if (chunks_in.size() > cfg_.max_chunks) throw std::runtime_error("too many chunks in batch");
  std::vector<size_t> order(chunks_in.size());
  for (size_t i = 0; i < order.size(); ++i) order[i] = i;
  std::stable_sort(order.begin(), order.end(), [&](size_t a, size_t b) {
    return files_[chunks_in[a].file].server < files_[chunks_in[b].file].server;
  });
  ps.chunk_file.assign(chunks_in.size(), 0);
  uint64_t off = 0;
  bool canonical = true;
  for (size_t k = 0; k < order.size(); ++k) {
    const Chunk& c = chunks_in[k];
    if (order[k] != k || c.begin != off) { canonical = false; break; }
    off = c.end;
  }
  canonical = canonical && off == n_bytes && n_bytes + 64 <= cfg_.max_batch_bytes + 256;
  ps.hb = ps.h_bytes;
  if (canonical) {
    ps.hb = host_bytes;
    for (size_t k = 0; k < order.size(); ++k) {
      const Chunk& c = chunks_in[k];
      if (c.end > c.begin && host_bytes[c.end - 1] != '\n') throw std::runtime_error("chunk must end with a newline");
      ps.h_chunk_begin[k] = (uint32_t)c.begin;
      ps.h_chunk_kind[k] = files_[c.file].kind;
      ps.h_chunk_file[k] = (uint32_t)c.file;
      ps.chunk_file[k] = c.file;
    }
  } else {
    off = 0;
    const bool in_place = host_bytes == ps.h_bytes;
    std::vector<uint8_t> tmp_copy;
    const uint8_t* src = host_bytes;
    if (in_place) {
      tmp_copy.assign(host_bytes, host_bytes + n_bytes);
      src = tmp_copy.data();
    }
    for (size_t k = 0; k < order.size(); ++k) {
      const Chunk& c = chunks_in[order[k]];
      const uint64_t len = c.end - c.begin;
      if (len > 0 && src[c.end - 1] != '\n') throw std::runtime_error("chunk must end with a newline");
      std::memcpy(ps.h_bytes + off, src + c.begin, len);
      ps.h_chunk_begin[k] = (uint32_t)off;
      ps.h_chunk_kind[k] = files_[c.file].kind;
      ps.h_chunk_file[k] = (uint32_t)c.file;
      ps.chunk_file[k] = c.file;
      off += len;
    }
    std::memset(ps.h_bytes + off, 0, 64);
  }
  const uint32_t n_chunks = (uint32_t)order.size();
  ps.h_chunk_begin[n_chunks] = (uint32_t)off;
  ps.n_bytes = off;
  ps.src = host_bytes;
  ps.src_n = n_bytes;
  metrics_.bytes += off;
  ++metrics_.batches;

  const int k = (int)(&ps - pslot_);
  bool staged = false;
  if (dev() && canonical && in_stage_src_ == host_bytes && in_stage_n_ == n_bytes && in_stage_ev_) {
    HIP_OK(hipStreamWaitEvent(parse_stream_, in_stage_ev_, 0));
    dj_->swap_stage(k);
    staged = true;
    ++metrics_.staged_batches;
  }
  in_stage_src_ = nullptr;
  in_stage_n_ = 0;
  uint8_t* dbytes = dev() ? dj_->d_bytes(k) : d_bytes_;
  Event* devents = dev() ? dj_->d_events(k) : d_events_;
  if (!staged) HIP_OK(hipMemcpyAsync(dbytes, ps.hb, off, hipMemcpyHostToDevice, parse_stream_));
  {
    CopySegs up;
    up.add(d_chunk_begin_[k], HipRes::device_alias(ps.h_chunk_begin), (size_t)(n_chunks + 1) * 4);
    up.add(d_chunk_kind_[k], HipRes::device_alias(ps.h_chunk_kind), n_chunks + 1);
    up.add(d_chunk_file_[k], HipRes::device_alias(ps.h_chunk_file), (size_t)(n_chunks + 1) * 4);
    if (dev()) {
      dj_->set_chunks(k, ps.chunk_file, d_chunk_file_[k], d_chunk_kind_[k]);
      dj_->chunk_upload(k, cfg_.max_lines, up);
    }
    apm_copy_segs(&up, parse_stream_);
  }
  if (apm_parse_batch(dbytes, off, d_chunk_begin_[k], d_chunk_kind_[k], d_chunk_file_[k], n_chunks, d_parse_ws_,
                      cfg_.max_lines, devents, d_counts_, d_counts_ + 1, d_watermark_, d_file_open_, &cfg_.tz,
                      parse_stream_) != 0)
    throw std::runtime_error("parse workspace too small");
  if (dev()) dj_->select_host(k, d_counts_, cfg_.max_lines, parse_stream_);
  {
    CopySegs ex;
    ex.add(HipRes::device_alias(ps.h_counts), d_counts_, 8);
    ex.add(HipRes::device_alias(ps.h_watermark), d_watermark_, 8);
    if (dev()) dj_->export_select(k, ex);
    apm_copy_segs(&ex, parse_stream_);
  }
  ps.spec_copied = 0;
  if (speculative && !dev() && spec_events_) {
    ps.spec_copied = std::min<uint32_t>(spec_events_, cfg_.max_lines);
    HIP_OK(hipMemcpyAsync(ps.h_events, d_events_, (size_t)ps.spec_copied * sizeof(Event), hipMemcpyDeviceToHost,
                          parse_stream_));
  }
  ps.pending = true;
  metrics_.t_parse_ms += now_ms() - t0;
}

void Engine::stage_batch(const uint8_t* host_bytes, uint64_t n_bytes) {
  if (!dev() || !host_bytes || n_bytes == 0 || n_bytes > cfg_.max_batch_bytes) return;
  const double t0 = now_ms();
  if (!in_stage_stream_) {
    HIP_OK(hipStreamCreateWithFlags(&in_stage_stream_, hipStreamNonBlocking));
    res_.adopt(in_stage_stream_);
    in_stage_ev_ = res_.new_event();
  }
  HIP_OK(hipMemcpyAsync(dj_->d_stage(), host_bytes, n_bytes, hipMemcpyHostToDevice, in_stage_stream_));
  HIP_OK(hipEventRecord(in_stage_ev_, in_stage_stream_));
  in_stage_src_ = host_bytes;
  in_stage_n_ = n_bytes;
  trace_event("stage H2D (launch)", t0, now_ms(), 0);
}

void Engine::finish_parse(ParseSlot& ps) {
  const double t0 = now_ms();
  HIP_OK(hipStreamSynchronize(parse_stream_));
  ps.n_events = ps.h_counts[0];
  ps.n_lines = ps.h_counts[1];
  if (ps.n_lines > cfg_.max_lines) throw std::runtime_error("batch has more lines than max_lines");
  metrics_.lines += ps.n_lines;
  metrics_.events += ps.n_events;
  if (!dev() && ps.n_events > ps.spec_copied) {
    const uint32_t lo = ps.spec_copied;
    HIP_OK(hipMemcpyAsync(ps.h_events + lo, d_events_ + lo, (size_t)(ps.n_events - lo) * sizeof(Event),
                          hipMemcpyDeviceToHost, parse_stream_));
    HIP_OK(hipStreamSynchronize(parse_stream_));
  }
  ps.spec_copied = 0;
  spec_events_ = ps.n_events + ps.n_events / 4 + 1024;
  ps.pending = false;
  last_slot_ = (int)(&ps - pslot_);
  metrics_.t_parse_ms += now_ms() - t0;
}

static void merge_shard_outputs(const std::vector<std::vector<TxOut>>& outs, bool multi, std::vector<TxOut>& txs) {
  txs.clear();
  const int ns = (int)outs.size();
  size_t total = 0;
  std::vector<size_t> split(ns, 0);
  for (int k = 0; k < ns; ++k) {
    auto& v = outs[k];
    total += v.size();
    size_t p = 0;
    while (p < v.size() && !(v[p].seq >> 63)) ++p;
    split[k] = p;
  }
  txs.reserve(total);
  using Item = std::pair<uint64_t, std::pair<int, size_t>>;
  std::priority_queue<Item, std::vector<Item>, std::greater<Item>> pq;
  for (int k = 0; k < ns; ++k)
    if (split[k] > 0) pq.push({outs[k][0].seq, {k, 0}});
  while (!pq.empty()) {
    auto it = pq.top();
    pq.pop();
    auto& v = outs[it.second.first];
    txs.push_back(v[it.second.second]);
    const size_t nx = it.second.second + 1;
    if (nx < split[it.second.first]) pq.push({v[nx].seq, {it.second.first, nx}});
  }
  std::vector<int> order;
  for (int k = 0; k < ns; ++k)
    if (split[k] < outs[k].size()) order.push_back(k);
  std::sort(order.begin(), order.end(), [&](int a, int b) { return outs[a][split[a]].seq < outs[b][split[b]].seq; });
  const size_t line_part = txs.size();
  for (int k : order) txs.insert(txs.end(), outs[k].begin() + (ptrdiff_t)split[k], outs[k].end());
  if (multi)
    std::stable_sort(txs.begin() + (ptrdiff_t)line_part, txs.end(),
                     [](const TxOut& a, const TxOut& b) { return a.seq < b.seq; });
}

void Engine::process_batch(const uint8_t* host_bytes, uint64_t n_bytes, const std::vector<Chunk>& chunks_in,
                           double now_override, const uint8_t* next_bytes, uint64_t next_n,
                           const std::vector<Chunk>* next_chunks) {
  const double t0 = now_ms();
  roctxRangePushA("apm.parse");
  ParseSlot& ps = pslot_[cur_slot_];
// ... 79 lines not shown
  {
    double sum = 0, mx = 0;
    for (size_t s = 0; s < shards_.size(); ++s) { sum += shard_ms_[s * 16]; mx = std::max(mx, shard_ms_[s * 16]); }
    metrics_.t_shard_busy_ms += shards_.empty() ? 0 : sum / shards_.size();
    metrics_.t_shard_max_ms += mx;
  }
  std::vector<std::vector<TxOut>> outs(shards_.size());
  {
    std::lock_guard<std::mutex> g(out_pool_mu_);
    for (size_t k = 0; k < shards_.size(); ++k) {
      outs[k].swap(shards_[k]->out());
      if (!out_pool_.empty()) {
        shards_[k]->out().swap(out_pool_.back());
        out_pool_.pop_back();
      }
    }
  }
  bool multi = false;
  for (auto& r : shard_range) multi |= r.size() > 1;
  const double t2 = now_ms();
  metrics_.t_join_ms += t2 - t1;
  metrics_.t_merge_ms += t2 - t1b;
  roctxRangePop();
  trace_event("join", t1, t1b, 0);
  trace_event("handoff", t1b, t2, 0);

  int sync_slot = -1;
  if (lockstep_) {
    int64_t bmax = INT64_MIN;
    for (size_t k = 0; k < shards_.size(); ++k) bmax = std::max(bmax, shard_maxb_[k * 8]);
    sync_slot = lockstep_collect(bmax);
  } else {
    watermark_ = batch_watermark(ps);
  }

  const double tp0 = now_ms();
  post_stats(std::move(outs), multi, t0, sync_slot);
  const double tp1 = now_ms();
  trace_event("post", tp0, tp1, 0);
  if (coll_) fleet_exchange_upto(fleet_posted_ - 1);
  trace_event("fleet.exchange", tp1, now_ms(), 0);
  metrics_.t_total_ms += now_ms() - t0;
  ++batch_no_;
}

void Engine::process_batch_dev_tail(ParseSlot& ps, double t0, double now_override, const uint8_t* next_bytes,
                                    uint64_t next_n, const std::vector<Chunk>* next_chunks) {
  const int k = (int)(&ps - pslot_);
  if (next_bytes && next_chunks) {
    launch_parse(pslot_[k ^ 1], next_bytes, next_n, *next_chunks, true);
    prefetched_ = true;
  }
  cur_slot_ = k ^ 1;
  last_n_events_ = ps.n_events;
  const double t1 = now_ms();
  roctxRangePop();
  roctxRangePushA("apm.join");
  trace_event("parse", t0, t1, 0);
  const double clock = now_override >= 0 ? now_override : watermark_;
  if (lockstep_) lockstep_issue(batch_watermark(ps));
  DevJoinBatch b;
  const DeviceJoin::ParallelFor par = [this](int n, const std::function<void(int)>& fn) { pool_->run(n, fn); };
  const std::function<void()> ahead = [this, k, par]() {
    if (!ahead_lane_) ahead_lane_.reset(new TaskLane());
    ahead_task_ = ahead_lane_->post([this, k, par]() {
      ParseSlot& nx = pslot_[k ^ 1];
      const double ta = now_ms();
      finish_parse(nx);
      dj_->prepass_ahead(k ^ 1, nx.hb, par);
      trace_event("next parse+prepass", ta, now_ms(), 3);
    });
  };
  const bool do_ahead = prefetched_;
  const std::function<void()> meanwhile = [this, &ahead, do_ahead]() {
    if (do_ahead) ahead();
    if (coll_ && fleet_due_ > fleet_rounds_) {
      const double tf = now_ms();
      fleet_exchange_upto(fleet_due_);
      trace_event("fleet.exchange", tf, now_ms(), 0);
    }
  };
  dj_->run(k, ps.hb, ps.n_events, ps.n_bytes, clock, batch_no_, want(OUT_TRANSACTIONS), want(OUT_AUDIT_DB), b, par,
           &meanwhile);
  const double t2 = now_ms();
  metrics_.t_join_ms += t2 - t1;
  metrics_.t_join_shards_ms += t2 - t1;
  metrics_.t_shard_max_ms += t2 - t1;
  metrics_.t_shard_busy_ms += t2 - t1;
  roctxRangePop();
  trace_event("join (GPU)", t1, t2, 0);
  if (trace_on_) {
    static const char* names[DeviceJoin::kPhases] = {"dj.prepass", "dj.upload", "dj.launch", "dj.syncA",
                                                     "dj.register", "dj.plan", "dj.write+syncC", "dj.tail"};
    for (int i = 0; i < DeviceJoin::kPhases; ++i) trace_event(names[i], dj_->phase_t[i], dj_->phase_t[i + 1], 2);
    for (const auto& sp : dj_->spans) trace_event(sp.first, sp.second.first, sp.second.second, 2);
  }
  const int sync_slot = lockstep_ ? lockstep_collect(b.max_bucket) : -1;
  if (!lockstep_) watermark_ = batch_watermark(ps);
  const double tp0 = now_ms();
  post_stats_dev(std::move(b), t0, sync_slot);
  const double tp1 = now_ms();
  trace_event("post", tp0, tp1, 0);
  if (coll_) fleet_due_ = fleet_posted_ - 1;
  metrics_.t_total_ms += now_ms() - t0;
  ++batch_no_;
}

void Engine::process_tx_lines(const std::string& blob, double now) {
  if (dev()) throw std::runtime_error("process_tx_lines needs gpu.joinOnDevice = false");
  const double t0 = now_ms();
  std::vector<std::vector<TxOut>> outs(shards_.size());
  uint64_t line = 0;
  size_t i = 0;
  while (i < blob.size()) {
    size_t j = blob.find('\n', i);
    if (j == std::string::npos) j = blob.size();
    const std::string_view ln(blob.data() + i, j - i);
    i = j + 1;
    if (ln.size() < 3 || ln.compare(0, 3, "tx|") != 0) continue;
    std::string_view f[9];
    int nf = 0;
    size_t a = 0;
    while (nf < 9) {
      const size_t b = ln.find('|', a);
      f[nf++] = ln.substr(a, b == std::string_view::npos ? std::string_view::npos : b - a);
      if (b == std::string_view::npos) break;
      a = b + 1;
    }
    if (nf < 8) { ++metrics_.tx_dropped; continue; }
    const std::string srv(f[1]);
    const auto known = server_ids_.find(srv);
    const int32_t sid = known != server_ids_.end() ? known->second : add_server(srv);
    if ((size_t)sid >= outs.size()) outs.resize(shards_.size());
    const int32_t svc = dict_.service_id(f[2]);
    std::string& arena = shards_[sid]->text();
    TxOut t{};
    t.seq = (1ULL << 63) | (line++ << 12);
    t.server = sid;
    t.service = svc;
    t.raw_svc = svc;
    t.end_ms = js::parse_int(f[6]);
    t.elapsed = js::parse_int(f[7]);
    t.line_off = (uint32_t)arena.size();
    t.line_len = (uint32_t)ln.size();
    t.to_db = false;
    t.toplevel = nf > 8 && f[8] == "Y";
    arena.append(ln.data(), ln.size());
    arena += '\n';
    outs[sid].push_back(t);
  }
  if (now >= 0 && now > watermark_) watermark_ = now;
  outs.resize(shards_.size());
  metrics_.lines += line;
  post_stats(std::move(outs), true, t0, -1);
  metrics_.t_total_ms += now_ms() - t0;
  ++batch_no_;
}

void Engine::trace_event(const char* name, double t0, double t1, int tid) {
  if (!trace_on_) return;
  std::lock_guard<std::mutex> g(trace_mu_);
  if (trace_.size() < 1000000) trace_.push_back(TraceEvent{name, t0, t1, tid, batch_no_});
}

std::vector<TraceEvent> Engine::take_trace() {
  flush();
// ... 2645 lines not shown
```

### apmbackend_amd/csrc/runtime/engine.h

```cpp
#pragma once
#include <hip/hip_runtime.h>

#include "binio.h"

#include <array>
#include <atomic>
#include <condition_variable>
#include <cstdint>
#include <deque>
#include <functional>
#include <map>
#include <memory>
#include <mutex>
#include <string>
#include <thread>
#include <tuple>
#include <unordered_map>
#include <vector>

#include "../apm_types.h"
#include "../kernels/kernel_api.h"
#include "collective.h"
#include "devjoin.h"
#include "hipres.h"
// ... 9 lines not shown
  double thr[MAX_LAGS] = {0, 0, 0, 0};
  double infl[MAX_LAGS] = {0, 0, 0, 0};
  double hard_max = 0;
  bool suppressed = false;
};

struct ReconfigSpec {
  uint64_t gen = 0;
  int n_lags = 0;
  int32_t lags[MAX_LAGS] = {0, 0, 0, 0};
  double thr[MAX_LAGS] = {0, 0, 0, 0};
  double infl[MAX_LAGS] = {0, 0, 0, 0};
  int lag_suppressed[MAX_LAGS] = {0, 0, 0, 0};
  int alert_window = 60, alert_threshold = 45, both_only = 1;
  double hard_min_ms = 200, hard_min_tpm = 1.0, hard_max_ms = 10000, cooldown_ms = 15 * 60000.0;
  int interval_len = 10, window = 30, buffer = 6;
  std::map<std::string, ServiceOverride> overrides;
};

void check_window(int window, int buffer, int interval_len);
int32_t ring_slots_for(int window, int buffer);

struct EngineConfig {
  int device = 0;
  int32_t max_series = 1 << 17;
  int32_t cell_cap = 16;
  int32_t spill_cap = 1 << 20;
  uint64_t max_batch_bytes = 64ull << 20;
  uint32_t max_lines = 1u << 21;
  uint32_t max_chunks = 4096;
  int64_t pool_cap = 1 << 23;
  int32_t max_tx_per_batch = 1 << 21;
  int32_t max_alerts = 1 << 16;
  int ring_bytes = 8;
  int exact_mean = 0;
  int sigma_stddev = 0;
  int resync_k = 360;
  bool resync_mfma = false;
  int n_lags = 2;
  int32_t lags[MAX_LAGS] = {360, 8640, 0, 0};
  double thr[MAX_LAGS] = {20.0, 15.0, 0, 0};
  double infl[MAX_LAGS] = {0.1, 0.0, 0, 0};
  int emulate_aliasing = 0;
  int alert_window = 60;
  int alert_threshold = 45;
  double hard_min_ms = 200;
  double hard_min_tpm = 1.0;
  double hard_max_ms = 10000;
  int both_only = 1;
  int lag_suppressed[MAX_LAGS] = {0, 0, 0, 0};
  double cooldown_ms = 15 * 60000.0;
  int cooldown_by_service = 1;
  int alert_clock_entry = 1;
  int interval_len = 10;
  int window = 30;
  int buffer = 6;
  int nslot = 0;
  int64_t ck_stage_bytes = (int64_t)2048 << 20;
  double record_ttl_ms = 120000, acct_ttl_ms = 120000, need_ttl_ms = 30000;
  TzTable tz{};
  int join_threads = 0;
  bool pin_threads = false;
  uint32_t outputs = 0;
  int32_t n_win_pcts = 0;
  int32_t win_pcts[8] = {0, 0, 0, 0, 0, 0, 0, 0};
  std::vector<std::vector<int64_t>> slo_classes;
  std::map<std::string, int32_t> slo_services;
  int32_t slo_default = 0;
  int32_t tk_k = 0;
  std::vector<int32_t> tk_by;
  double tk_min_tpm = 0.0;
  int32_t n_svc_pcts = 0;
  int32_t svc_pcts[8] = {0, 0, 0, 0, 0, 0, 0, 0};
  int async_stats = 1;
  double coll_timeout_ms = 300000;
  double coll_init_timeout_ms = 120000;
  int node_cooldown = 1;
  int device_join = 1;
  int join_table_bits = 21;
  uint32_t need_arena = 1u << 18;
  uint32_t join_chain_blocks = 0;
  uint64_t tx_ring_bytes = 4ull << 30;
  uint32_t max_raw_services = 1u << 20;
};

enum OutKind { OUT_TRANSACTIONS = 0, OUT_AUDIT_DB, OUT_DB, OUT_ST, OUT_FS, OUT_AL, OUT_SX, OUT_FB, OUT_LH, OUT_WP, OUT_SL, OUT_TK, OUT_SV, N_OUT };
constexpr int N_OUT_CKPT = OUT_FB + 1;
constexpr uint32_t kLaneKinds = (1u << OUT_DB) | (1u << OUT_ST) | (1u << OUT_FS) | (1u << OUT_LH) | (1u << OUT_WP) |
                                (1u << OUT_SL) | (1u << OUT_TK) | (1u << OUT_SV);
const char* out_kind_name(int k);
int out_kind_of(const std::string& name);

struct BucketDump {
  int64_t latest = 0;
  std::vector<int32_t> series;
  std::vector<int64_t> bucket;
  std::vector<int32_t> count;
  std::vector<int32_t> values;
};

struct TraceEvent {
  const char* name;
  double t0_ms, t1_ms;
  int tid;
  uint64_t batch;
};

struct Chunk {
  int32_t file;
  uint64_t begin, end;
};

struct ByteSink {
  virtual ~ByteSink() = default;
  virtual void write_bytes(int kind, const char* p, size_t n) = 0;
  virtual void write_bytes_held(int kind, const char* p, size_t n, std::shared_ptr<const void> hold) {
    (void)hold;
    write_bytes(kind, p, n);
  }
  virtual void write_rows_held(int kind, const char* p, size_t n, const uint32_t* row_off, size_t nrows,
                               std::shared_ptr<const void> hold) {
    (void)row_off;
    (void)nrows;
    write_bytes_held(kind, p, n, std::move(hold));
  }
};

struct CheckpointInfo {
  bool busy = false;
  uint64_t done = 0, skipped = 0, sync_fallbacks = 0;
  int chain_len = 0;
  bool last_base = false;
  double last_stall_ms = 0, last_write_ms = 0;
  uint64_t last_bytes = 0, stage_bytes = 0;
  int64_t last_ring_rows = 0;
  uint64_t last_deferred_bytes = 0;
  uint64_t streamed = 0, streamed_live_rows = 0, side_rows = 0, guard_stalls = 0;
  uint64_t stage_cap = 0;
};

struct EngineMetrics {
  uint64_t batches = 0, bytes = 0, lines = 0, events = 0, tx = 0, tx_db = 0, tx_dropped = 0;
  uint64_t rollovers = 0, alerts = 0, alert_candidates = 0, series = 0, released = 0;
  uint64_t staged_batches = 0;
  uint64_t alert_candidates_dropped = 0;
  uint64_t formatted_bytes = 0, format_fallbacks = 0, lockstep_rollovers = 0;
  uint64_t series_overflow_tx = 0;
  uint64_t spill_dropped = 0;
  uint64_t nan_windows_clipped = 0;
  uint64_t tx_capacity_grows = 0;
  uint64_t spill_grows = 0;
  int64_t spill_capacity = 0;
  double t_parse_ms = 0, t_join_ms = 0, t_stats_ms = 0, t_total_ms = 0;
  double t_join_shards_ms = 0, t_merge_ms = 0;
  double t_shard_busy_ms = 0, t_shard_max_ms = 0;
  double t_stats_tx_ms = 0, t_rollover_ms = 0, t_format_ms = 0, t_release_ms = 0;
  double t_out_ms = 0;
  uint64_t db_copy_rows = 0, db_copy_fallbacks = 0;
  double t_lockstep_ms = 0, t_lockstep_max_ms = 0;
  double t_lockstep_stats_ms = 0;
  std::vector<double> rollover_latency_ms;
};

void pin_current_thread(int cpu);
std::vector<int> local_core_slice(int device);

class ThreadPool {
 public:
  explicit ThreadPool(int n, const std::vector<int>& cpus = {});
  ~ThreadPool();
  void run(int n_tasks, const std::function<void(int)>& fn, const std::function<void()>* meanwhile = nullptr);
  int size() const { return (int)workers_.size(); }

 private:
  std::vector<std::thread> workers_;
  std::mutex mu_;
  std::condition_variable cv_, done_cv_;
  const std::function<void(int)>* fn_ = nullptr;
  int n_tasks_ = 0, done_ = 0;
  uint64_t gen_ = 0;
  bool stop_ = false;
};

class TaskLane {
 public:
  TaskLane();
  ~TaskLane();
  uint64_t post(std::function<void()> fn);
  void wait(uint64_t id);
  void wait_all();

 private:
  std::thread th_;
  std::mutex mu_;
  std::condition_variable cv_;
  std::deque<std::function<void()>> q_;
  uint64_t posted_ = 0, done_ = 0;
  std::string err_;
  bool stop_ = false;
};

class Engine {
 public:
  explicit Engine(const EngineConfig& cfg);
  ~Engine();

  int32_t add_server(const std::string& name);
  int32_t add_file(const std::string& path, int kind, const std::string& server);
  void set_override(const std::string& service, const ServiceOverride& o);
  void clear_overrides();
  void refresh_series_settings();
  void stage_reconfig(const ReconfigSpec& spec);
  uint64_t reconfig_applied_gen() const { return rc_applied_gen_.load(); }
  uint64_t reconfigs_applied() const { return reconfigs_applied_.load(); }
  uint64_t lag_set_changes() const { return lag_set_changes_.load(); }
  uint64_t window_changes() const { return window_changes_.load(); }
  int32_t ring_slots() const { return nslot_; }
  uint64_t ring_grows() const { return ring_grows_; }
  std::vector<int32_t> lag_values() { flush(); return std::vector<int32_t>(cfg_.lags, cfg_.lags + cfg_.n_lags); }

  void process_batch(const uint8_t* host_bytes, uint64_t n_bytes, const std::vector<Chunk>& chunks,
                     double now_override = -1.0, const uint8_t* next_bytes = nullptr, uint64_t next_n = 0,
                     const std::vector<Chunk>* next_chunks = nullptr);
  bool prefetch_pending() const { return prefetched_; }
  void stage_batch(const uint8_t* host_bytes, uint64_t n_bytes);
  void process_tx_lines(const std::string& blob, double now = -1.0);

// ... 334 lines not shown
  void ser_tab_put(int32_t server, int32_t service, int32_t s) {
    if (server < 0 || service < 0 || service >= (1 << 20)) return;
    if ((size_t)server >= ser_tab_.size()) ser_tab_.resize((size_t)server + 1);
    auto& row = ser_tab_[server];
    if ((size_t)service >= row.size()) row.resize(std::max<size_t>((size_t)service + 1, row.size() * 2), -1);
    row[service] = s;
  }
  std::vector<SeriesInfo> series_;
  int32_t n_series_ = 0;
  std::vector<int32_t> server_rank_;
  std::vector<int32_t> server_next_service_;
  int32_t next_server_rank_ = 0;
  std::map<std::string, ServiceOverride> overrides_;
  double alias_thr_[MAX_LAGS], alias_infl_[MAX_LAGS];
  std::vector<double> h_thr_, h_infl_, h_hard_max_;
  std::vector<uint8_t> h_suppressed_;
  std::vector<uint64_t> h_emit_key_;
  std::vector<int32_t> zscore_seen_;
  std::vector<uint8_t> h_active_;
  std::vector<int32_t> unseen_;

  std::unique_ptr<DeviceJoin> dj_;
  const DevJoinBatch* cur_dj_ = nullptr;
  uint64_t ring_low_pending_ = UINT64_MAX;
  unsigned long long* d_ring_min_ = nullptr;
  Mapped<unsigned long long> h_ring_min_;
  int64_t* d_rel_n_ = nullptr;
  Mapped<int64_t> h_rel_n_;
  uint32_t* d_rel_lens_ = nullptr;
  uint32_t* d_rel_offs_ = nullptr;
  uint32_t* d_rel_fb_ = nullptr;
  Mapped<uint32_t> h_rel_total_;
  char* d_rel_text_[2] = {nullptr, nullptr};
  size_t rel_text_cap_[2] = {0, 0};
  PinnedBuf<char> h_rel_text_[REL_RING];
  int rel_ring_k_ = 0;
  PinnedBuf<uint32_t> h_rel_offs_[2];
  hipStream_t out_stream_ = nullptr;
  std::vector<int32_t> h_raw_series_;
  static constexpr int kStage = 32;
  PinnedBuf<char> h_stage_[kStage];
  size_t stage_max_ = 0;
  hipEvent_t stage_ev_[kStage] = {};
  int stage_k_ = 0;
  void h2d(void* d, const void* h_pinned, size_t n, hipStream_t s);
  void d2h(void* h_pinned, const void* d, size_t n, hipStream_t s);
  char* stage(size_t bytes);
  void stage_done();
  int32_t* d_pairs_ = nullptr;
  size_t pairs_bytes_ = 0;
  int32_t* pinned_pairs(size_t n_ints);
  void pinned_pairs_done() { stage_done(); }
  size_t max_name_len_ = 0;
  int32_t* d_unseen_idx_ = nullptr;
  uint8_t* d_unseen_flag_ = nullptr;
  uint8_t* h_unseen_flag_ = nullptr;
  unsigned long long* d_unmapped_ = nullptr;
  bool dev() const { return dj_ != nullptr; }

  uint8_t* d_bytes_ = nullptr;
  struct ParseSlot {
    uint8_t* h_bytes = nullptr;
    uint32_t* h_chunk_begin = nullptr;
    uint8_t* h_chunk_kind = nullptr;
    uint32_t* h_chunk_file = nullptr;
    Event* h_events = nullptr;
    uint32_t* h_counts = nullptr;
    unsigned long long* h_watermark = nullptr;
    const uint8_t* hb = nullptr;
    const uint8_t* src = nullptr;
    uint64_t src_n = 0, n_bytes = 0;
    std::vector<int32_t> chunk_file;
    uint32_t n_events = 0, n_lines = 0;
    uint32_t spec_copied = 0;
    bool pending = false;
  } pslot_[2];
  uint32_t spec_events_ = 0;
  int cur_slot_ = 0, last_slot_ = 0;
  bool prefetched_ = false;
  const uint8_t* in_stage_src_ = nullptr;
  uint64_t in_stage_n_ = 0;
  hipStream_t in_stage_stream_ = nullptr;
  hipEvent_t in_stage_ev_ = nullptr;
  void launch_parse(ParseSlot& ps, const uint8_t* host_bytes, uint64_t n_bytes, const std::vector<Chunk>& chunks,
                    bool speculative = false);
  void process_batch_dev_tail(ParseSlot& ps, double t0, double now_override, const uint8_t* next_bytes,
                              uint64_t next_n, const std::vector<Chunk>* next_chunks);
  void finish_parse(ParseSlot& ps);
  double batch_watermark(const ParseSlot& ps) const;
  uint32_t* d_chunk_begin_[2] = {nullptr, nullptr};
  uint8_t* d_chunk_kind_[2] = {nullptr, nullptr};
  uint32_t* d_chunk_file_[2] = {nullptr, nullptr};
  void* d_parse_ws_ = nullptr;
  Event* d_events_ = nullptr;
  uint32_t* d_counts_ = nullptr;
  unsigned long long* d_watermark_ = nullptr;
  uint8_t* d_file_open_ = nullptr;
  TzTable* d_tz_unused_ = nullptr;

  int32_t* d_counts_cells_ = nullptr;
  int32_t* d_cells_ = nullptr;
  int32_t* d_spill_n_ = nullptr;
  int32_t* d_spill_series_ = nullptr;
  int32_t* d_spill_val_ = nullptr;
  int32_t* d_spill_series_alt_ = nullptr;
  int32_t* d_spill_val_alt_ = nullptr;
  void* d_spill_tmp_ = nullptr;
  size_t spill_tmp_bytes_ = 0;
  Mapped<int32_t> h_spill_snap_;
  uint64_t spill_added_ = 0;
  std::vector<uint64_t> spill_clear_at_;
  struct SpillMark { hipEvent_t ev = nullptr; uint64_t added = 0; bool live = false; };
  static constexpr int kSpillMarks = 4;
  SpillMark spill_mark_[kSpillMarks];
  int spill_mark_k_ = 0;
  void spill_reserve(uint32_t n);
  void spill_marked();
  void spill_resync();
  void grow_spill(int32_t cap);
  void spill_sort();
  unsigned long long* d_spill_drop_ = nullptr;
  uint8_t* d_active_ = nullptr;
  int32_t nslot_ = NSLOT_MIN;
  std::vector<int64_t> slot_bucket_;
  uint64_t ring_grows_ = 0;
  int32_t* d_win_slots_ = nullptr;
  void alloc_ring(int32_t nslot);
  void grow_ring(int32_t nslot);
  int64_t latest_ = 0;
  int64_t rollover_idx_ = 0;
  WinStat* d_win_ = nullptr;
  int32_t* d_big_list_ = nullptr;
  int32_t* d_big_n_ = nullptr;
  int32_t* d_nan_until_ = nullptr;
  int32_t* d_ord_list_ = nullptr;
  int32_t* d_ord_n_ = nullptr;
  int32_t* d_nan_list_ = nullptr;
  int32_t* d_nan_n_ = nullptr;
  int32_t* d_js_scratch_ = nullptr;
  static constexpr int32_t kJsCap = 1 << 18;
  StatsState stats_state() const;
  void grow_tx_capacity(uint32_t need, uint32_t keep);
  int64_t ord_cap_ = 0;

  struct CkJob {
    struct Lag { int32_t n_cols = 0; std::vector<int32_t> heads; size_t off = 0; };
    bool streamed = false;
    bool base = false;
    int64_t seq = 0;
    std::string prefix, name, path, extra;
    MemBlob blob;
    std::vector<Lag> lags;
    std::function<void()> pre_commit;
    std::vector<std::array<size_t, 3>> holes;
    std::vector<std::pair<size_t, int32_t>> patches;
  };
  static constexpr int kMaxChain = 16;
  enum : uint8_t { CKR_NONE = 0, CKR_LIVE, CKR_READING, CKR_STAGED, CKR_SIDE, CKR_DONE };
  struct CkStream {
    bool on = false;
    std::vector<std::vector<uint8_t>> state;
    std::vector<std::vector<size_t>> off;
    size_t side_used = 0, side_cap = 0;
    bool side_sync = false;
    int32_t n_cols = 0;
    uint64_t live_rows = 0, side_rows = 0, stalls = 0;
// ... 334 lines not shown
```

### apmbackend_amd/models/pipeline.py

```python
from __future__ import annotations

import logging
import math
import os
import time
from typing import Any, Dict, Iterable, List, Optional, Sequence, Tuple, Union

from .. import _native
from ..models.oracle import file_kind, server_of
from ..ops.parse_ref import tz_table
from ..utils.config import (LEADERBOARD_KEYS, latency_objectives, leaderboard, service_window, slo_tables,
                            window_percentiles)
from ..utils.timeparse import TzOffset

log = logging.getLogger("apm.pipeline")

KIND_CODE = {"SOAP": 0, "SERVER": 1, "APP": 2}

OUT_KINDS = ("transactions", "audit_db", "db", "st", "fs", "al", "sx", "fb", "lh")
ALL_OUT_KINDS = OUT_KINDS + ("wp",)
ENGINE_OUT_KINDS = ALL_OUT_KINDS + ("sl",)
NATIVE_OUT_KINDS = ENGINE_OUT_KINDS + ("tk",)
DEVICE_OUT_KINDS = NATIVE_OUT_KINDS + ("sv",)
KEEP_TEXT_KINDS = tuple(k for k in OUT_KINDS if k != "lh")
DB_OUTPUTS = ("audit_db", "db", "fs", "al")
MAX_LAGS = 16


def output_mask(kinds) -> int:
    m = 0
    for k in kinds:
        m |= 1 << DEVICE_OUT_KINDS.index(k)
    return m


def engine_config(cfg: Dict[str, Any], device: int = 0, keep_text: bool = False, outputs=None,
                  tz: Optional[TzOffset] = None, tz_centre_ms: Optional[int] = None, **kw) -> Dict[str, Any]:
    g = cfg.get("gpu", {})
    win_pcts = window_percentiles(cfg)
    if "wp" in (outputs or ()) and not win_pcts:
        raise ValueError('outputs names "wp" but gpu.windowPercentiles is empty')
    slo_classes, slo_services, slo_default = slo_tables(latency_objectives(cfg))
    if "sl" in (outputs or ()) and not slo_classes:
        raise ValueError('outputs names "sl" but gpu.latencyObjectives holds no threshold')
    board = leaderboard(cfg)
    if "tk" in (outputs or ()) and not board:
        raise ValueError('outputs names "tk" but gpu.leaderboard is not set')
    svc_pcts = service_window(cfg)
    if "sv" in (outputs or ()) and not svc_pcts:
        raise ValueError('outputs names "sv" but gpu.serviceWindow is not set')
    zc = cfg["streamCalcZScore"]
    ac = cfg["streamProcessAlerts"]
    sc = cfg["streamCalcStats"]
    lags = sorted(((int(d["LAG"]), float(d["THRESHOLD"]), float(d["INFLUENCE"])) for d in zc["defaults"]),
                  key=lambda x: x[0])
    if len(lags) > MAX_LAGS:
        raise ValueError(f"at most {MAX_LAGS} LAG settings are supported per engine")
    suppressed_lags = {int(x) for x in ac.get("suppressedLags", [])}
    ring = {"float64": 8, "float32": 4, "bfloat16": 2, "bf16": 2}.get(g.get("ringDtype", "float64"), 8)
    if tz is None:
        tz = TzOffset(g.get("timezone", "local"))
    d = {
        "device": device,
        "max_series": int(g.get("maxSeries", 1 << 17)),
        "cell_cap": int(g.get("bucketCellCapacity", 16)),
        "spill_cap": int(g.get("bucketOverflowCapacity", 1 << 22)) // 40 or 1,
        "max_batch_bytes": int(g.get("batchBytes", 32 << 20)) * 2,
        "max_lines": min(int(g.get("maxLinesPerBatch", 1 << 20)) * 2, (1 << 21) - 1),
        "max_tx_per_batch": int(g.get("maxTxPerBatch", int(g.get("maxLinesPerBatch", 1 << 20)) * 2)),
        "ring_bytes": ring,
        "exact_mean": 1 if g.get("zscoreMeanMode", "rolling") == "exact" else 0,
        "sigma_stddev": 1 if g.get("zscoreSigma", "sqrt_mean") == "stddev" else 0,
        "resync_k": int(g.get("exactRecomputeEveryIntervals", 360)),
        "resync_mfma": bool(g.get("resyncOnMatrixCores", False)),
        "emulate_aliasing": 1 if g.get("emulateOverrideAliasing", False) else 0,
        "lags": lags,
        "lag_suppressed": [1 if l[0] in suppressed_lags else 0 for l in lags],
        "alert_window": int(ac["rollingAlertWindowSizeInIntervals"]),
        "alert_threshold": int(ac["requiredNumberBadIntervalsInAlertWindowToTrigger"]),
        "hard_min_ms": float(ac["hardMinMsAlertThreshold"]),
        "hard_min_tpm": float(ac["hardMinTpmAlertThreshold"]),
        "hard_max_ms": float(ac["hardMaxMsAlertThreshold"]),
        "both_only": 1 if ac.get("alertOnBothOnly") else 0,
        "cooldown_ms": float(ac["perServiceAlertCooldownInMinutes"]) * 60000.0,
        "cooldown_by_service": 1 if g.get("cooldownKey", "service") == "service" else 0,
        "alert_clock_entry": 1 if g.get("alertClock", "entry") == "entry" else 0,
        "interval_len": int(sc["intervalLengthInSeconds"]),
        "window": int(sc["windowSizeInIntervals"]),
        "nslot": int(g.get("bucketRingSlots", 0)),
        "ck_stage_bytes": int(float(g.get("checkpointStageMB", 2048)) * (1 << 20)),
        "buffer": int(sc["bufferSizeInIntervals"]),
        "record_ttl_ms": float(g.get("recordTtlSeconds", 120)) * 1000.0,
        "acct_ttl_ms": float(g.get("acctTtlSeconds", 120)) * 1000.0,
        "need_ttl_ms": float(g.get("needTtlSeconds", 30)) * 1000.0,
        "tz_table": tz_table(tz, tz_centre_ms),
        "join_threads": int(g.get("joinThreads", 0)),
        "pin_threads": bool(g.get("pinThreads", False)),
        "coll_timeout_ms": float(g.get("collectiveTimeoutSeconds", 300)) * 1000.0,
        "coll_init_timeout_ms": float(g.get("collectiveInitTimeoutSeconds", 120)) * 1000.0,
        "node_cooldown": 1 if g.get("nodeCooldown", True) else 0,
        "device_join": 1 if g.get("joinOnDevice", True) else 0,
        "join_table_bits": max(10, (int(g.get("joinTableSlots", 1 << 21)) - 1).bit_length()),
        "need_arena": int(g.get("needArenaEntries", 1 << 18)),
        "join_chain_blocks": int(g.get("joinChainBlocks", 0)),
        "tx_ring_bytes": min(int(g.get("txTextRingMB", 4096)), max(256, (128 * int(g.get("batchBytes", 32 << 20))) >> 20)) << 20,
        "max_raw_services": max(int(g.get("maxRawServices", 1 << 18)), 2 * int(g.get("maxSeries", 1 << 17))),
        "outputs": output_mask(KEEP_TEXT_KINDS if keep_text else ()) | output_mask(outputs or ()),
        "win_pcts": win_pcts,
        "slo_classes": slo_classes,
        "slo_services": slo_services,
        "slo_default": slo_default,
        "tk_k": board["k"] if board else None,
        "tk_by": [LEADERBOARD_KEYS.index(b) for b in board["by"]] if board else [],
        "tk_min_tpm": board["minTpm"] if board else 0.0,
        "svc_pcts": svc_pcts,
    }
    w, b = d["window"], d["buffer"]
    if not (w >= 1 and b >= 0 and d["interval_len"] >= 1):
        raise ValueError(f"stats window: windowSizeInIntervals >= 1, bufferSizeInIntervals >= 0, "
                         f"intervalLengthInSeconds >= 1 (got {w} / {b} / {d['interval_len']})")
    d.update(kw)
    return d


def service_overrides(cfg: Dict[str, Any]) -> Dict[str, Dict[str, Any]]:
    zc = cfg["streamCalcZScore"]
    ac = cfg["streamProcessAlerts"]
    lags = sorted(int(d["LAG"]) for d in zc["defaults"])
    out: Dict[str, Dict[str, Any]] = {}
    for svc, per_lag in ((zc.get("overrides") or {}).get("services") or {}).items():
        o = out.setdefault(svc, {"thr": [None] * len(lags), "infl": [None] * len(lags)})
        for lag_key, vals in per_lag.items():
            try:
                li = lags.index(int(float(lag_key)))
            except ValueError:
                continue
            if "THRESHOLD" in vals:
                o["thr"][li] = float(vals["THRESHOLD"])
            if "INFLUENCE" in vals:
                o["infl"][li] = float(vals["INFLUENCE"])
    for svc, vals in ((ac.get("overrides") or {}).get("services") or {}).items():
        o = out.setdefault(svc, {"thr": [None] * len(lags), "infl": [None] * len(lags)})
        hm = vals.get("hardMaxMsAlertThreshold")
        if hm:
            o["hard_max"] = float(hm)
    for svc in ac.get("suppressedServices", []) or []:
        o = out.setdefault(svc, {"thr": [None] * len(lags), "infl": [None] * len(lags)})
        o["suppressed"] = True
    return out


_last_gen = [0]


def _reload_generation(cfg: Dict[str, Any]) -> int:
    path = cfg.get("apmConfigFilePath")
    g = 0
    if path and os.path.exists(path):
        g = os.stat(path).st_mtime_ns // 1_000_000
    if g <= 0:
        g = _last_gen[0] + 1
    _last_gen[0] = max(_last_gen[0], g)
    return g


class APMEngine:
    def __init__(self, cfg: Dict[str, Any], device: int = 0, keep_text: bool = False, outputs=None,
                 tz: Optional[TzOffset] = None, tz_centre_ms: Optional[int] = None, **kw):
        self.cfg = cfg
        self.N = _native.load()
        self.tz = tz if tz is not None else TzOffset(cfg.get("gpu", {}).get("timezone", "local"))
        self.tz_centre_ms = int(time.time() * 1000) if tz_centre_ms is None else int(tz_centre_ms)
        self.ecfg = engine_config(cfg, device, keep_text, outputs, tz=self.tz, tz_centre_ms=self.tz_centre_ms, **kw)
        self.eng = self.N.Engine(self.ecfg)
        self.file_ids: Dict[str, int] = {}
        self.apply_overrides(cfg)

    def apply_overrides(self, cfg: Dict[str, Any]):
        self.eng.clear_overrides()
        for svc, o in service_overrides(cfg).items():
            self.eng.set_override(svc, o)

    LIVE_KEYS = ("lags", "lag_suppressed", "alert_window", "alert_threshold", "hard_min_ms", "hard_min_tpm",
                 "hard_max_ms", "both_only", "cooldown_ms", "interval_len", "window", "buffer")

    @classmethod
    def restart_required(cls, old: Dict[str, Any], new: Dict[str, Any]) -> List[str]:
# ... 97 lines not shown
```

### apmbackend_amd/utils/config.py

```python
from __future__ import annotations

import copy
import decimal
import hashlib
import json
import logging
import math
import os
import re
import threading
import time
from typing import Any, Callable, Dict, Iterable, List, Optional, Tuple

log = logging.getLogger("apm.config")

_STRIP_RE = re.compile(r"[^:]//(.*)")

DEFAULT_CONFIG_PATH = os.path.join(
    os.path.dirname(os.path.dirname(os.path.dirname(os.path.abspath(__file__)))),
    "config", "apm_config.json")

GPU_DEFAULTS: Dict[str, Any] = {
    "device": 0,
    "maxSeries": 1 << 17,
    "maxServices": 1 << 16,
    "maxServers": 1024,
    "bucketCellCapacity": 16,
    "bucketRingSlots": 0,
    "bucketOverflowCapacity": 1 << 22,
    "batchBytes": 32 << 20,
    "maxLinesPerBatch": 1 << 20,
    "ringDtype": "float64",
    "pinThreads": False,
    "zscoreMeanMode": "rolling",
    "zscoreSigma": "sqrt_mean",
    "exactRecomputeEveryIntervals": 360,
    "emulateOverrideAliasing": False,
    "alertClock": "wall",
    "cooldownKey": "service",
    "recordTtlSeconds": 120,
    "acctTtlSeconds": 120,
    "needTtlSeconds": 30,
    "timezone": "local",
    "fleetBaseline": True,
    "joinThreads": 0,
    "joinOnDevice": True,
    "joinTableSlots": 1 << 21,
    "needArenaEntries": 1 << 18,
    "joinChainBlocks": 0,
    "txTextRingMB": 4096,
    "maxRawServices": 1 << 18,
    "collectiveTimeoutSeconds": 300,
    "collectiveInitTimeoutSeconds": 120,
    "collectiveBackend": "rccl",
    "checkpointDir": "",
    "checkpointEverySeconds": 60,
    "checkpointStageMB": 2048,
    "importReferenceResume": False,
    "outputMode": "inproc",
    "bridgeQueues": [],
    "tailFromStart": False,
    "serverRollup": False,
    "fuseJmx": False,
    "syntheticJmx": False,
    "logFilePrefix": "apm_engine",
    "faultInjection": {},
}

GPU_OPTIONAL: Dict[str, Any] = {
    "latencyHistogram": False,
    "histQueue": "latency_hist",
    "windowPercentiles": [],
    "pctQueue": "window_pct",
    "latencyObjectives": None,
    "sloQueue": "window_slo",
    "leaderboard": None,
    "topQueue": "leaderboard",
    "serviceWindow": None,
    "svcQueue": "service_window",
}

def gpu_opt(cfg: Dict[str, Any], key: str) -> Any:
    return (cfg.get("gpu") or {}).get(key, GPU_OPTIONAL[key])


MAX_WINDOW_PCTS = 8
PCT_SCALE = 100000


def parse_window_percentiles(v: Any) -> List[int]:
    if v is None:
        return []
    if isinstance(v, (str, bytes)) or not isinstance(v, (list, tuple)):
        raise ValueError(f"gpu.windowPercentiles: a list of percentiles, got {v!r}")
    if len(v) > MAX_WINDOW_PCTS:
        raise ValueError(f"gpu.windowPercentiles: at most {MAX_WINDOW_PCTS} percentiles, got {len(v)}")
    out: List[int] = []
    for p in v:
        if isinstance(p, bool) or not isinstance(p, (int, float, str, decimal.Decimal)):
            raise ValueError(f"gpu.windowPercentiles: {p!r} is not a number")
        try:
            d = decimal.Decimal(repr(p) if isinstance(p, float) else str(p).strip())
        except decimal.InvalidOperation:
            raise ValueError(f"gpu.windowPercentiles: {p!r} is not a number") from None
        if not d.is_finite():
            raise ValueError(f"gpu.windowPercentiles: {p!r} is not finite")
        q = d * 1000
        if q != q.to_integral_value():
            raise ValueError(f"gpu.windowPercentiles: {p!r} has more than three decimals")
        q = int(q)
        if not 1 <= q <= PCT_SCALE:
            raise ValueError(f"gpu.windowPercentiles: {p!r} is outside (0, 100]")
        if out and q <= out[-1]:
            raise ValueError(f"gpu.windowPercentiles: {p!r} does not ascend strictly")
        out.append(q)
    return out


def window_percentiles(cfg: Dict[str, Any]) -> List[int]:
    return parse_window_percentiles(gpu_opt(cfg, "windowPercentiles"))


MAX_SLO_THRESHOLDS = 8
SLO_T_MAX = 2147483647


def _parse_threshold_list(where: str, v: Any) -> List[int]:
    if not isinstance(v, (list, tuple)):
        raise ValueError(f"gpu.latencyObjectives: {where} must be a list of integers, got {v!r}")
    if len(v) > MAX_SLO_THRESHOLDS:
        raise ValueError(f"gpu.latencyObjectives: {where} holds {len(v)} thresholds, at most {MAX_SLO_THRESHOLDS}")
    out: List[int] = []
    for t in v:
        if isinstance(t, bool) or not isinstance(t, int):
            raise ValueError(f"gpu.latencyObjectives: {where}: {t!r} is not an integer")
        if not 0 <= t <= SLO_T_MAX:
            raise ValueError(f"gpu.latencyObjectives: {where}: {t!r} is outside 0 .. {SLO_T_MAX}")
        if out and t <= out[-1]:
            raise ValueError(f"gpu.latencyObjectives: {where}: {t!r} does not ascend strictly")
        out.append(t)
    return out


def parse_latency_objectives(v: Any) -> Optional[Dict[str, Any]]:
    if v is None:
        return None
    if not isinstance(v, dict):
        raise ValueError(f"gpu.latencyObjectives: an object with 'default' and / or 'services', got {v!r}")
    extra = set(v) - {"default", "services"}
    if extra:
        raise ValueError(f"gpu.latencyObjectives: unknown key(s) {sorted(extra)!r}")
    default = _parse_threshold_list("default", v["default"]) if v.get("default") is not None else []
    services = v.get("services")
    if services is None:
        services = {}
    if not isinstance(services, dict):
        raise ValueError(f"gpu.latencyObjectives: services must be an object, got {services!r}")
    named: Dict[str, List[int]] = {}
    for name, lst in services.items():
        if not isinstance(name, str):
            raise ValueError(f"gpu.latencyObjectives: service name {name!r} is not a string")
        named[name] = _parse_threshold_list(f"services[{name!r}]", lst)
# ... 239 lines not shown
```

Before: 324.4 million.

## Slice batch upload and line-split parse so H2D copy overlaps parsing

Adds an optional slice plan that splits each batch's host-to-device byte copy into aligned slices on a separate copy stream. Each slice records an event, and the newline count, tile scan, line write and line parse kernels for that slice wait on it. The aim is to hide upload time behind parsing. The rocprim device scan over tile counts is replaced by a single-block incremental scan kernel that also writes the line count, and the parse kernel no longer zeroes keep flags past the line count. Slicing is off by default (parseSliceBytes=0), but the new scan kernel and parse bounds apply on every path. The single-block scan may be slower for large tile counts, and the cross-stream events add ordering overhead.

Result: slower. 312.2 million (-3.8%).

```diff
diff --git a/apmbackend_amd/csrc/bindings.cpp b/apmbackend_amd/csrc/bindings.cpp
--- a/apmbackend_amd/csrc/bindings.cpp
+++ b/apmbackend_amd/csrc/bindings.cpp
@@ -148,6 +148,7 @@
   c.join_table_bits = get<int>(d, "join_table_bits", c.join_table_bits);
   c.need_arena = get<uint32_t>(d, "need_arena", c.need_arena);
   c.join_chain_blocks = get<uint32_t>(d, "join_chain_blocks", c.join_chain_blocks);
+  c.parse_slice_bytes = get<uint64_t>(d, "parse_slice_bytes", c.parse_slice_bytes);
   c.tx_ring_bytes = get<uint64_t>(d, "tx_ring_bytes", c.tx_ring_bytes);
   c.max_raw_services = get<uint32_t>(d, "max_raw_services", c.max_raw_services);
   return c;
@@ -184,6 +185,7 @@
   d["alerts"] = m.alerts; d["alert_candidates"] = m.alert_candidates;
   d["alert_candidates_dropped"] = m.alert_candidates_dropped; d["released"] = m.released;
   d["staged_batches"] = m.staged_batches;
+  d["sliced_batches"] = m.sliced_batches;
   d["t_join_shards_ms"] = m.t_join_shards_ms; d["t_merge_ms"] = m.t_merge_ms;
   d["t_shard_busy_ms"] = m.t_shard_busy_ms; d["t_shard_max_ms"] = m.t_shard_max_ms;
   d["t_out_ms"] = m.t_out_ms;
@@ -827,6 +829,12 @@
   m.def("js_to_fixed", [](double x, int f) { return js::to_fixed(x, f); });
   m.def("js_num_str", [](double x) { return js::num_str(x); });
   m.def("js_parse_int", [](const std::string& s) { return js::parse_int(s); });
+  m.def("parse_slice_ranges", [](uint64_t n_bytes, uint64_t slice_bytes) {
+    const ApmSlicePlan p = apm_parse_slice_plan(n_bytes, slice_bytes);
+    std::vector<std::pair<uint64_t, uint64_t>> r;
+    for (uint32_t s = 0; s < p.n; ++s) r.emplace_back(s * p.slice, std::min<uint64_t>((s + 1) * p.slice, n_bytes));
+    return r;
+  }, py::arg("n_bytes"), py::arg("slice_bytes"));
   m.def("js_convert_date", [](const std::string& s, const py::dict& tz) {
     double v;
     TzTable t = tz_from(tz);
diff --git a/apmbackend_amd/csrc/kernels/kernel_api.h b/apmbackend_amd/csrc/kernels/kernel_api.h
--- a/apmbackend_amd/csrc/kernels/kernel_api.h
+++ b/apmbackend_amd/csrc/kernels/kernel_api.h
@@ -311,11 +311,18 @@
 
 extern "C" {
 size_t apm_parse_workspace_bytes(uint64_t max_bytes, uint32_t max_lines, uint32_t max_chunks);
+constexpr uint32_t APM_PARSE_SLICE_ALIGN = 16384;
+constexpr uint32_t APM_PARSE_MAX_SLICES = 32;
+struct ApmSlicePlan {
+  uint32_t n;
+  uint64_t slice;
+};
+ApmSlicePlan apm_parse_slice_plan(uint64_t n_bytes, uint64_t slice_bytes);
 int apm_parse_batch(const uint8_t* d_bytes, uint64_t n_bytes, const uint32_t* d_chunk_begin,
                     const uint8_t* d_chunk_kind, const uint32_t* d_chunk_file, uint32_t n_chunks,
                     void* d_ws, uint32_t max_lines, apm::Event* d_events, uint32_t* d_n_events,
                     uint32_t* d_n_lines, unsigned long long* d_watermark, uint8_t* d_file_open,
-                    const apm::TzTable* tz, hipStream_t stream);
+                    const apm::TzTable* tz, ApmSlicePlan plan, const hipEvent_t* ready, hipStream_t stream);
 size_t apm_ck_pack_tmp_bytes(uint64_t n_entries);
 int apm_ck_pack_cells(const int32_t* counts, const int32_t* cells, const int32_t* d_slots, int k, int32_t n, int32_t S,
                       int32_t cap, uint32_t* lens, uint32_t* offs, void* tmp, size_t tmp_bytes, int32_t* packed,
diff --git a/apmbackend_amd/csrc/kernels/parse.hip b/apmbackend_amd/csrc/kernels/parse.hip
--- a/apmbackend_amd/csrc/kernels/parse.hip
+++ b/apmbackend_amd/csrc/kernels/parse.hip
@@ -32,14 +32,14 @@
 
 __global__ __launch_bounds__(NL_BLOCK) void k_nl_count(const uint8_t* __restrict__ bytes, uint64_t n,
                                                       uint32_t* __restrict__ tile_counts, uint8_t* __restrict__ pad,
-                                                      uint32_t tiles) {
-  if (blockIdx.x == 0 && threadIdx.x < 64) pad[threadIdx.x] = 0;
-  if (blockIdx.x == 0 && threadIdx.x == 64) tile_counts[tiles] = 0;
+                                                      uint32_t blk0, uint32_t tiles) {
+  if (pad && blockIdx.x == 0 && threadIdx.x < 64) pad[threadIdx.x] = 0;
+  const uint32_t blk = blk0 + blockIdx.x;
   uint4 v[NL_PER];
   uint64_t base[NL_PER];
 #pragma unroll
   for (int k = 0; k < NL_PER; ++k) {
-    base[k] = ((uint64_t)blockIdx.x * NL_PER + k) * NL_TILE + threadIdx.x * 16;
+    base[k] = ((uint64_t)blk * NL_PER + k) * NL_TILE + threadIdx.x * 16;
     if (base[k] + 16 <= n) v[k] = *reinterpret_cast<const uint4*>(bytes + base[k]);
   }
   uint32_t pk[NL_PER / 2] = {0, 0};
@@ -65,27 +65,59 @@
     const int k = threadIdx.x;
     uint32_t sum = 0;
     for (int i = 0; i < NL_BLOCK / APM_WAVE; ++i) sum += red[k >> 1][i];
-    const uint32_t tile = blockIdx.x * NL_PER + k;
+    const uint32_t tile = blk * NL_PER + k;
     if (tile < tiles) tile_counts[tile] = (sum >> (16 * (k & 1))) & 0xFFFFu;
+  }
+}
+
+constexpr int TS_BLOCK = 1024, TS_ITEMS = 4;
+__global__ __launch_bounds__(TS_BLOCK) void k_tile_scan(const uint32_t* __restrict__ tile_counts,
+                                                       uint32_t* __restrict__ tile_off, uint32_t t0, uint32_t t1,
+                                                       uint32_t* __restrict__ n_lines) {
+  typedef rocprim::block_scan<uint32_t, TS_BLOCK> Scan;
+  __shared__ typename Scan::storage_type st;
+  uint32_t carry = t0 ? tile_off[t0] : 0u;
+  for (uint32_t b = t0; b < t1; b += TS_BLOCK * TS_ITEMS) {
+    const uint32_t j0 = b + threadIdx.x * TS_ITEMS;
+    uint32_t v[TS_ITEMS];
+    uint32_t lane = 0;
+#pragma unroll
+    for (int k = 0; k < TS_ITEMS; ++k) {
+      v[k] = j0 + k < t1 ? tile_counts[j0 + k] : 0u;
+      lane += v[k];
+    }
+    uint32_t excl, sum;
+    Scan().exclusive_scan(lane, excl, 0u, sum, st);
+    excl += carry;
+#pragma unroll
+    for (int k = 0; k < TS_ITEMS; ++k) {
+      if (j0 + k < t1) tile_off[j0 + k] = excl;
+      excl += v[k];
+    }
+    carry += sum;
+    __syncthreads();
+  }
+  if (threadIdx.x == 0) {
+    tile_off[t1] = carry;
+    *n_lines = carry;
   }
 }
 
 __global__ __launch_bounds__(NL_BLOCK) void k_nl_write(const uint8_t* __restrict__ bytes, uint64_t n,
                                                       const uint32_t* __restrict__ tile_off,
-                                                      uint32_t* __restrict__ line_end, uint32_t* __restrict__ n_lines,
-                                                      uint32_t tiles) {
-  if (blockIdx.x == 0 && threadIdx.x == 0) *n_lines = tile_off[tiles];
+                                                      uint32_t* __restrict__ line_end, uint32_t blk0, uint32_t tiles) {
+  const uint32_t blk = blk0 + blockIdx.x;
   uint4 v[NL_PER];
 #pragma unroll
   for (int k = 0; k < NL_PER; ++k) {
-    const uint64_t base = ((uint64_t)blockIdx.x * NL_PER + k) * NL_TILE + threadIdx.x * 16;
+    const uint64_t base = ((uint64_t)blk * NL_PER + k) * NL_TILE + threadIdx.x * 16;
     v[k] = base + 16 <= n ? *reinterpret_cast<const uint4*>(bytes + base) : make_uint4(0, 0, 0, 0);
   }
   typedef rocprim::block_scan<int, NL_BLOCK> Scan;
   __shared__ typename Scan::storage_type st;
 #pragma unroll
   for (int k = 0; k < NL_PER; ++k) {
-    const uint32_t tile = blockIdx.x * NL_PER + k;
+    const uint32_t tile = blk * NL_PER + k;
     if (tile >= tiles) break;
     const uint64_t base = (uint64_t)tile * NL_TILE + threadIdx.x * 16;
     uint8_t b[16];
@@ -274,6 +306,8 @@
   const uint32_t* chunk_begin;
   const uint8_t* chunk_kind;
   const uint32_t* n_lines_dev;
+  const uint32_t* line_lo;
+  const uint32_t* line_hi;
   uint32_t cap_lines;
   uint32_t n_chunks;
   Event* ev_tmp;
@@ -377,13 +411,9 @@
   __shared__ __attribute__((aligned(16))) uint8_t lds[PARSE_LDS];
   __shared__ uint16_t tok_lds[2 * NTOKSLOT][PARSE_BLOCK];
   long long pt = a.prof ? clock64() : 0;
-  const uint32_t n_lines = *a.n_lines_dev;
-  const uint32_t first = blockIdx.x * PARSE_BLOCK;
-  if (first >= n_lines) {
-    const uint32_t li = first + threadIdx.x;
-    if (li < a.cap_lines) a.keep[li] = 0;
-    return;
-  }
+  const uint32_t n_lines = min(*a.line_hi, a.cap_lines);
+  const uint32_t first = (a.line_lo ? *a.line_lo : 0u) + blockIdx.x * PARSE_BLOCK;
+  if (first >= n_lines) return;
   const uint32_t last = min(first + PARSE_BLOCK, n_lines);
   const uint32_t r0 = first == 0 ? 0 : a.line_end[first - 1] + 1;
   const uint32_t r1 = a.line_end[last - 1] + 1;
@@ -411,9 +441,7 @@
   pprof(a, PP_STAGE, pt);
   const uint32_t li = first + threadIdx.x;
   unsigned long long wm = 0;
-  if (li >= last) {
-    if (li < a.cap_lines) a.keep[li] = 0;
-  } else {
+  if (li < last) {
     const uint32_t ls = li == 0 ? 0 : a.line_end[li - 1] + 1;
     const uint32_t le = a.line_end[li];
     const uint32_t c_lo = find_chunk(a.chunk_begin, a.n_chunks, r0), c_hi = find_chunk(a.chunk_begin, a.n_chunks, r1 - 1);
@@ -1053,19 +1081,34 @@
   return b;
 }
 
+ApmSlicePlan apm_parse_slice_plan(uint64_t n_bytes, uint64_t slice_bytes) {
+  const uint64_t A = APM_PARSE_SLICE_ALIGN;
+  uint64_t slice = (slice_bytes + A - 1) / A * A;
+  if (slice == 0 || slice >= n_bytes) return {1u, n_bytes};
+  if ((n_bytes + slice - 1) / slice > APM_PARSE_MAX_SLICES)
+    slice = ((n_bytes + APM_PARSE_MAX_SLICES - 1) / APM_PARSE_MAX_SLICES + A - 1) / A * A;
+  return {(uint32_t)((n_bytes + slice - 1) / slice), slice};
+}
+
 int apm_parse_batch(const uint8_t* d_bytes, uint64_t n_bytes, const uint32_t* d_chunk_begin,
                     const uint8_t* d_chunk_kind, const uint32_t* d_chunk_file, uint32_t n_chunks,
                     void* d_ws, uint32_t max_lines, apm::Event* d_events, uint32_t* d_n_events,
                     uint32_t* d_n_lines, unsigned long long* d_watermark, uint8_t* d_file_open,
-                    const apm::TzTable* tz, hipStream_t stream) {
+                    const apm::TzTable* tz, ApmSlicePlan plan, const hipEvent_t* ready, hipStream_t stream) {
   using namespace apm;
+  static_assert(APM_PARSE_SLICE_ALIGN == (uint32_t)NL_PER * NL_TILE, "a slice boundary is a block boundary of K1");
   const uint32_t tiles = (uint32_t)((n_bytes + NL_TILE - 1) / NL_TILE);
   if (tiles == 0 || n_chunks == 0) {
+    if (ready)
+      for (uint32_t s = 0; s < plan.n; ++s) HIP_OK(hipStreamWaitEvent(stream, ready[s], 0));
     HIP_OK(hipMemsetAsync(d_n_events, 0, 4, stream));
     HIP_OK(hipMemsetAsync(d_n_lines, 0, 4, stream));
     HIP_OK(hipMemsetAsync(const_cast<uint8_t*>(d_bytes) + n_bytes, 0, 64, stream));
     return 0;
   }
+  if (plan.n == 0 || plan.n > APM_PARSE_MAX_SLICES || (plan.n > 1 && plan.slice % APM_PARSE_SLICE_ALIGN != 0) ||
+      (uint64_t)plan.n * plan.slice < n_bytes || (uint64_t)(plan.n - 1) * plan.slice >= n_bytes)
+    return -1;
   const uint32_t cap = (uint32_t)std::min<uint64_t>(max_lines, n_bytes);
   uint8_t* w = (uint8_t*)d_ws;
   auto carve = [&](size_t bytes) { uint8_t* r = (uint8_t*)(((uintptr_t)w + 63) & ~(uintptr_t)63); w = r + bytes; return r; };
@@ -1079,16 +1122,6 @@
   uint32_t* chunk_line_lo = (uint32_t*)carve((size_t)(n_chunks + 2) * 4);
   uint8_t* seg_state = carve((size_t)(n_chunks + 2) * SEC_SEGS);
   uint8_t* chunk_init = carve((size_t)(n_chunks + 2));
-  void* scan_tmp = carve(APM_SCAN_TMP);
-
-  const uint32_t nl_blocks = (tiles + NL_PER - 1) / NL_PER;
-  hipLaunchKernelGGL(k_nl_count, dim3(nl_blocks), dim3(NL_BLOCK), 0, stream, d_bytes, n_bytes, tile_counts,
-                     const_cast<uint8_t*>(d_bytes) + n_bytes, tiles);
-  PrimScratch sc(scan_tmp, APM_SCAN_TMP);
-  if (prim_exclusive_scan(sc, tile_counts, tile_off, 0u, (size_t)tiles + 1, rocprim::plus<uint32_t>(), stream) != 0)
-    return -1;
-  hipLaunchKernelGGL(k_nl_write, dim3(nl_blocks), dim3(NL_BLOCK), 0, stream, d_bytes, n_bytes, tile_off, line_end,
-                     d_n_lines, tiles);
 
   ParseArgs pa;
   pa.bytes = d_bytes;
@@ -1096,6 +1129,7 @@
   pa.chunk_begin = d_chunk_begin;
   pa.chunk_kind = d_chunk_kind;
   pa.n_lines_dev = d_n_lines;
+  pa.line_lo = pa.line_hi = nullptr;
   pa.cap_lines = cap;
   pa.n_chunks = n_chunks;
   pa.ev_tmp = ev_tmp;
@@ -1113,10 +1147,27 @@
   pa.prof = prof_on ? d_prof : nullptr;
   const char* mode_env = getenv("APM_PARSE");
   const bool by_line = !(mode_env && strcmp(mode_env, "tile") == 0);
-  if (by_line)
-    hipLaunchKernelGGL(k_parse_lines, dim3((cap + PARSE_BLOCK - 1) / PARSE_BLOCK), dim3(PARSE_BLOCK), 0,
-                       stream, pa);
-  else
+  for (uint32_t s = 0; s < plan.n; ++s) {
+    const uint64_t b0 = (uint64_t)s * plan.slice, b1 = std::min<uint64_t>(b0 + plan.slice, n_bytes);
+    const uint32_t t0 = (uint32_t)(b0 / NL_TILE), t1 = (uint32_t)((b1 + NL_TILE - 1) / NL_TILE);
+    const uint32_t blk0 = t0 / NL_PER, nl_blocks = (t1 - t0 + NL_PER - 1) / NL_PER;
+    const bool last_slice = s + 1 == plan.n;
+    if (ready) HIP_OK(hipStreamWaitEvent(stream, ready[s], 0));
+    hipLaunchKernelGGL(k_nl_count, dim3(nl_blocks), dim3(NL_BLOCK), 0, stream, d_bytes, b1, tile_counts,
+                       last_slice ? const_cast<uint8_t*>(d_bytes) + n_bytes : (uint8_t*)nullptr, blk0, t1);
+    hipLaunchKernelGGL(k_tile_scan, dim3(1), dim3(TS_BLOCK), 0, stream, (const uint32_t*)tile_counts, tile_off, t0,
+                       t1, d_n_lines);
+    hipLaunchKernelGGL(k_nl_write, dim3(nl_blocks), dim3(NL_BLOCK), 0, stream, d_bytes, b1,
+                       (const uint32_t*)tile_off, line_end, blk0, t1);
+    if (by_line) {
+      pa.line_lo = t0 ? tile_off + t0 : nullptr;
+      pa.line_hi = tile_off + t1;
+      const uint32_t slice_cap = (uint32_t)std::min<uint64_t>(cap, b1 - b0);
+      hipLaunchKernelGGL(k_parse_lines, dim3((slice_cap + PARSE_BLOCK - 1) / PARSE_BLOCK), dim3(PARSE_BLOCK), 0,
+                         stream, pa);
+    }
+  }
+  if (!by_line)
     hipLaunchKernelGGL(k_parse_tiles, dim3(tiles), dim3(APM_WAVE), 0, stream, pa, n_bytes, (const uint32_t*)tile_off);
   if (prof_on && ++prof_batches % 50 == 0) {
     unsigned long long h[PP_N];
diff --git a/apmbackend_amd/csrc/runtime/devjoin.h b/apmbackend_amd/csrc/runtime/devjoin.h
--- a/apmbackend_amd/csrc/runtime/devjoin.h
+++ b/apmbackend_amd/csrc/runtime/devjoin.h
@@ -63,6 +63,7 @@
   }
   void swap_stage(int k) { std::swap(sl_[k].d_bytes, d_stage_bytes_); }
   Event* d_events(int k) { return sl_[k].d_events; }
+  hipStream_t stream() const { return stream_; }
   void select_host(int k, const uint32_t* d_n_ev, uint32_t max_ev, hipStream_t ps);
   void set_chunks(int k, const std::vector<int32_t>& chunk_file, const uint32_t* d_chunk_file,
                   const uint8_t* d_chunk_kind);
diff --git a/apmbackend_amd/csrc/runtime/engine.cpp b/apmbackend_amd/csrc/runtime/engine.cpp
--- a/apmbackend_amd/csrc/runtime/engine.cpp
+++ b/apmbackend_amd/csrc/runtime/engine.cpp
@@ -269,6 +269,8 @@
   }
   ev_a_ = res_.new_event();
   ev_b_ = res_.new_event();
+  parse_done_ev_ = res_.new_event();
+  join_done_ev_ = res_.new_event();
   const int32_t S = cfg_.max_series;
   if (cfg_.device_join) {
     DevJoinConfig dc;
@@ -523,6 +525,7 @@
   }
   ahead_lane_.reset();
   if (in_stage_stream_) hipStreamSynchronize(in_stage_stream_);
+  if (copy_stream_) hipStreamSynchronize(copy_stream_);
   fb_lane_.reset();
   if (nm_ev_) hipEventSynchronize(nm_ev_);
   checkpoint_shutdown();
@@ -849,7 +852,25 @@
   in_stage_n_ = 0;
   uint8_t* dbytes = dev() ? dj_->d_bytes(k) : d_bytes_;
   Event* devents = dev() ? dj_->d_events(k) : d_events_;
-  if (!staged) HIP_OK(hipMemcpyAsync(dbytes, ps.hb, off, hipMemcpyHostToDevice, parse_stream_));
+  const ApmSlicePlan plan = apm_parse_slice_plan(off, cfg_.parse_slice_bytes);
+  const bool sliced = !staged && plan.n > 1;
+  if (sliced) {
+    if (!copy_stream_) {
+      HIP_OK(hipStreamCreateWithFlags(&copy_stream_, hipStreamNonBlocking));
+      res_.adopt(copy_stream_);
+      for (hipEvent_t& e : slice_ev_) e = res_.new_event();
+    }
+    if (parse_done_set_) HIP_OK(hipStreamWaitEvent(copy_stream_, parse_done_ev_, 0));
+    if (join_done_set_) HIP_OK(hipStreamWaitEvent(copy_stream_, join_done_ev_, 0));
+    for (uint32_t s = 0; s < plan.n; ++s) {
+      const uint64_t b0 = s * plan.slice, b1 = std::min<uint64_t>(b0 + plan.slice, off);
+      HIP_OK(hipMemcpyAsync(dbytes + b0, ps.hb + b0, b1 - b0, hipMemcpyHostToDevice, copy_stream_));
+      HIP_OK(hipEventRecord(slice_ev_[s], copy_stream_));
+    }
+    ++metrics_.sliced_batches;
+  } else if (!staged) {
+    HIP_OK(hipMemcpyAsync(dbytes, ps.hb, off, hipMemcpyHostToDevice, parse_stream_));
+  }
   {
     CopySegs up;
     up.add(d_chunk_begin_[k], HipRes::device_alias(ps.h_chunk_begin), (size_t)(n_chunks + 1) * 4);
@@ -862,9 +883,9 @@
     apm_copy_segs(&up, parse_stream_);
   }
   if (apm_parse_batch(dbytes, off, d_chunk_begin_[k], d_chunk_kind_[k], d_chunk_file_[k], n_chunks, d_parse_ws_,
-                      cfg_.max_lines, devents, d_counts_, d_counts_ + 1, d_watermark_, d_file_open_, &cfg_.tz,
-                      parse_stream_) != 0)
-    throw std::runtime_error("parse workspace too small");
+                      cfg_.max_lines, devents, d_counts_, d_counts_ + 1, d_watermark_, d_file_open_, &cfg_.tz, plan,
+                      sliced ? slice_ev_ : nullptr, parse_stream_) != 0)
+    throw std::runtime_error("parse: slice plan does not fit the batch");
   if (dev()) dj_->select_host(k, d_counts_, cfg_.max_lines, parse_stream_);
   {
     CopySegs ex;
@@ -878,6 +899,10 @@
     ps.spec_copied = std::min<uint32_t>(spec_events_, cfg_.max_lines);
     HIP_OK(hipMemcpyAsync(ps.h_events, d_events_, (size_t)ps.spec_copied * sizeof(Event), hipMemcpyDeviceToHost,
                           parse_stream_));
+  }
+  if (cfg_.parse_slice_bytes) {
+    HIP_OK(hipEventRecord(parse_done_ev_, parse_stream_));
+    parse_done_set_ = true;
   }
   ps.pending = true;
   metrics_.t_parse_ms += now_ms() - t0;
@@ -1123,6 +1148,10 @@
   };
   dj_->run(k, ps.hb, ps.n_events, ps.n_bytes, clock, batch_no_, want(OUT_TRANSACTIONS), want(OUT_AUDIT_DB), b, par,
            &meanwhile);
+  if (cfg_.parse_slice_bytes) {
+    HIP_OK(hipEventRecord(join_done_ev_, dj_->stream()));
+    join_done_set_ = true;
+  }
   const double t2 = now_ms();
   metrics_.t_join_ms += t2 - t1;
   metrics_.t_join_shards_ms += t2 - t1;
diff --git a/apmbackend_amd/csrc/runtime/engine.h b/apmbackend_amd/csrc/runtime/engine.h
--- a/apmbackend_amd/csrc/runtime/engine.h
+++ b/apmbackend_amd/csrc/runtime/engine.h
@@ -115,6 +115,7 @@
   uint32_t join_chain_blocks = 0;
   uint64_t tx_ring_bytes = 4ull << 30;
   uint32_t max_raw_services = 1u << 20;
+  uint64_t parse_slice_bytes = 0;
 };
 
 enum OutKind { OUT_TRANSACTIONS = 0, OUT_AUDIT_DB, OUT_DB, OUT_ST, OUT_FS, OUT_AL, OUT_SX, OUT_FB, OUT_LH, OUT_WP, OUT_SL, OUT_TK, OUT_SV, N_OUT };
@@ -176,6 +177,7 @@
   uint64_t batches = 0, bytes = 0, lines = 0, events = 0, tx = 0, tx_db = 0, tx_dropped = 0;
   uint64_t rollovers = 0, alerts = 0, alert_candidates = 0, series = 0, released = 0;
   uint64_t staged_batches = 0;
+  uint64_t sliced_batches = 0;
   uint64_t alert_candidates_dropped = 0;
   uint64_t formatted_bytes = 0, format_fallbacks = 0, lockstep_rollovers = 0;
   uint64_t series_overflow_tx = 0;
@@ -676,6 +678,10 @@
   uint64_t in_stage_n_ = 0;
   hipStream_t in_stage_stream_ = nullptr;
   hipEvent_t in_stage_ev_ = nullptr;
+  hipStream_t copy_stream_ = nullptr;
+  hipEvent_t slice_ev_[APM_PARSE_MAX_SLICES] = {};
+  hipEvent_t parse_done_ev_ = nullptr, join_done_ev_ = nullptr;
+  bool parse_done_set_ = false, join_done_set_ = false;
   void launch_parse(ParseSlot& ps, const uint8_t* host_bytes, uint64_t n_bytes, const std::vector<Chunk>& chunks,
                     bool speculative = false);
   void process_batch_dev_tail(ParseSlot& ps, double t0, double now_override, const uint8_t* next_bytes,
diff --git a/apmbackend_amd/models/pipeline.py b/apmbackend_amd/models/pipeline.py
--- a/apmbackend_amd/models/pipeline.py
+++ b/apmbackend_amd/models/pipeline.py
@@ -9,7 +9,7 @@
 from .. import _native
 from ..models.oracle import file_kind, server_of
 from ..ops.parse_ref import tz_table
-from ..utils.config import (LEADERBOARD_KEYS, latency_objectives, leaderboard, service_window, slo_tables,
+from ..utils.config import (GPU_OPTIONAL, LEADERBOARD_KEYS, latency_objectives, leaderboard, service_window, slo_tables,
                             window_percentiles)
 from ..utils.timeparse import TzOffset
 
@@ -103,6 +103,7 @@
         "join_table_bits": max(10, (int(g.get("joinTableSlots", 1 << 21)) - 1).bit_length()),
         "need_arena": int(g.get("needArenaEntries", 1 << 18)),
         "join_chain_blocks": int(g.get("joinChainBlocks", 0)),
+        "parse_slice_bytes": max(0, int(g.get("parseSliceBytes", GPU_OPTIONAL["parseSliceBytes"]))),
         "tx_ring_bytes": min(int(g.get("txTextRingMB", 4096)), max(256, (128 * int(g.get("batchBytes", 32 << 20))) >> 20)) << 20,
         "max_raw_services": max(int(g.get("maxRawServices", 1 << 18)), 2 * int(g.get("maxSeries", 1 << 17))),
         "outputs": output_mask(KEEP_TEXT_KINDS if keep_text else ()) | output_mask(outputs or ()),
diff --git a/apmbackend_amd/utils/config.py b/apmbackend_amd/utils/config.py
--- a/apmbackend_amd/utils/config.py
+++ b/apmbackend_amd/utils/config.py
@@ -78,6 +78,7 @@
     "topQueue": "leaderboard",
     "serviceWindow": None,
     "svcQueue": "service_window",
+    "parseSliceBytes": 0,
 }
 
 def gpu_opt(cfg: Dict[str, Any], key: str) -> Any:
```
